# feiyuhuahuo/Yolact_minimal

Hardware: AMD Instinct MI355X
Metric: img/s res101_coco 544x544 inference (bs=1/GPU, 4 requests in flight) (higher is better)
Workload: dtype f32; 1 GPU; res101_coco 544x544 (the reference's "550-class" size) bs=1 inference: forward + nms + after_nms(480x640) per image, 4 independent bs=1 requests in flight on 4 HIP streams; global_batch=1, parallelism=replicas x1 (inference does not shard), weights=seeded random init, post_inputs=synthetic dense head outputs (17.8k candidates), requests_in_flight=4

## Files before the change

yolact_minimal_amd/csrc/conv_common.h:

```cpp
#pragma once
#include <cstdlib>
#include "ym_common.h"

namespace ymk {

constexpr int BK = 32;

struct FastDiv {
    unsigned mg, sh, d;
    __host__ static FastDiv make(unsigned d) {
        if (d == 0) d = 1;
        unsigned s = 0;
        while ((1ull << s) < d) ++s;
        return FastDiv{(unsigned)(((1ull << 32) * ((1ull << s) - d)) / d + 1), s, d};
    }
    __device__ __forceinline__ unsigned div(unsigned x) const { return (__umulhi(x, mg) + x) >> sh; }
    __device__ __forceinline__ void divmod(unsigned x, unsigned& q, unsigned& r) const { q = div(x); r = x - q * d; }
};

typedef int i32x4_t __attribute__((ext_vector_type(4)));
constexpr unsigned OOB = 0xFFFFFFF0u;
__device__ __forceinline__ f32x4 buf_ld16(__amdgpu_buffer_rsrc_t r, unsigned byte_off) {
    return __builtin_bit_cast(f32x4, __builtin_amdgcn_raw_buffer_load_b128(r, (int)byte_off, 0, 0));
}
__device__ __forceinline__ f32x4 buf_ld16_s(__amdgpu_buffer_rsrc_t r, unsigned byte_off, int soffset) {
    return __builtin_bit_cast(f32x4, __builtin_amdgcn_raw_buffer_load_b128(r, (int)byte_off, soffset, 0));
}
template <int I> struct IC { static constexpr int value = I; };
template <int I, int N, class F>
__device__ __forceinline__ void static_for(F&& f) {
    if constexpr (I < N) { f(IC<I>{}); static_for<I + 1, N>(f); }
}
constexpr int AUX_SC1 = 16;
__device__ __forceinline__ f32x4 buf_ld16_sc1(__amdgpu_buffer_rsrc_t r, unsigned byte_off) {
    return __builtin_bit_cast(f32x4, __builtin_amdgcn_raw_buffer_load_b128(r, (int)byte_off, 0, AUX_SC1));
}
__device__ __forceinline__ void buf_st16_sc1(__amdgpu_buffer_rsrc_t r, unsigned byte_off, f32x4 v) {
    __builtin_amdgcn_raw_buffer_store_b128(__builtin_bit_cast(i32x4_t, v), r, (int)byte_off, 0, AUX_SC1);
}

struct SegDev {
    float* out;
    long long bstride;
    int n0, n1, pitch, act;
};

struct ConvP {
    const float* in;
    const float* w;
    const float* scale;
    const float* shift;
    const float* residual;
    float* ws;
    double* bn_sum;
    double* bn_sumsq;
    const float* bnb_y;
    const float* bnb_out;
    const float* bnb_mean;
    const float* bnb_invstd;
    const float* bnb_gamma;
    const float* bnb_beta;
    int bnb_relu;
    int bn_ordered;
    int* counters;
    int B, H, W, Cin, Cout, KH, KW, stride, pad, Ho, Wo, Kpad;
    int M, HoWo, nkt, ksplit, kt_per_split, tiles_m, tiles_n;
    int main_blocks, main_tiles, tail_split, tail_ktps;
    FastDiv fd_ksplit, fd_tail, fd_tiles_n, fd_howo, fd_wo, fd_cin, fd_kw;
    int nlev;
    int lev_h[5], lev_w[5], lev_m[6], lev_pix[6];
    int cls;
    int M_pix;
    int cls_tile0[5];
    int cls_rows[4];
    int cls_w[4];
    FastDiv cls_fd_hw[4], cls_fd_w[4];
    int cls_kh0[4], cls_kw0[4], cls_nkw[4];
    int cls_nkt[4], cls_ktps[4], cls_tail_ktps[4];
    int n_groups;
    FastDiv fd_grp, fd_gn, fd_gn_last;
    long long* trace;
    const int* trace_epoch;
    int trace_ring;
    int trace_stride;
    int trace_rt;
    int* trace_hw;
    unsigned in_bytes, w_bytes, ws_bytes;
    int total_items;
    int nseg;
    int vec;
    SegDev seg[3];
};

__device__ __forceinline__ void ym_tile_decode(const ConvP& p, int id, int& tile_m, int& tile_n) {
    const unsigned g = p.fd_grp.div((unsigned)id);
    const unsigned r = (unsigned)id - g * p.fd_grp.d;
    const bool last = (int)g == p.n_groups - 1;
    const unsigned w = last ? p.fd_gn_last.d : p.fd_gn.d;
    const unsigned tm = last ? p.fd_gn_last.div(r) : p.fd_gn.div(r);
    tile_m = (int)tm;
    tile_n = (int)(g * p.fd_gn.d + (r - tm * w));
}

inline void ym_set_tile_order(ConvP& p, int groups, bool allow_model) {
    const int tn = p.tiles_n > 0 ? p.tiles_n : 1, tm = p.tiles_m > 0 ? p.tiles_m : 1;
    static const char* env = getenv("YM_TILE_GROUPS");
    if (groups <= 0) {
        const double a = (double)p.in_bytes, w = (double)p.w_bytes;
        if (env && env[0] == 'l') groups = (allow_model && w > a) ? tn : 1;
        else if (env && atoi(env) > 0) groups = allow_model ? atoi(env) : 1;
        else {
            groups = 1;
            double best = a + 8.0 * w;
            const bool small = a + w <= 8.0 * 1024 * 1024;
            if (allow_model && !small && w > a) groups = tn;
            for (int g = 2; g <= 8 && allow_model && small; g *= 2) {
                if (tn < g) break;
                const double t = g * a + (8.0 / g) * w;
                if (t < 0.95 * best) { best = t; groups = g; }
            }
        }
    }
    if (groups > tn) groups = tn;
    const int gw = (tn + groups - 1) / groups;
    p.n_groups = (tn + gw - 1) / gw;
    p.fd_gn = FastDiv::make((unsigned)gw);
    p.fd_gn_last = FastDiv::make((unsigned)(tn - (p.n_groups - 1) * gw));
    p.fd_grp = FastDiv::make((unsigned)(tm * gw));
}

#ifdef YM_TRACE
__device__ __forceinline__ size_t ym_trace_region(const ConvP& p) {
    if (!p.trace_epoch) return 0;
    const unsigned e = (unsigned)__hip_atomic_load(p.trace_epoch, __ATOMIC_RELAXED, __HIP_MEMORY_SCOPE_AGENT);
    return (size_t)(e % (unsigned)p.trace_ring) * (p.trace_stride ? (unsigned)p.trace_stride : gridDim.x);
}
#define YM_STAMP(i) do { if ((i) == 3) __builtin_amdgcn_s_waitcnt(0); if (p.trace && threadIdx.x == 0) { const size_t reg_ = ym_trace_region(p); p.trace[(reg_ + blockIdx.x) * 4 + (i)] = (long long)((p.trace_epoch || p.trace_rt) ? __builtin_amdgcn_s_memrealtime() : __builtin_amdgcn_s_memtime()) | ((i) == 0 ? (long long)(__builtin_amdgcn_s_getreg(0x1814) & 15) << 60 : 0ll); if ((i) == 0 && p.trace_hw) p.trace_hw[reg_ + blockIdx.x] = (int)__builtin_amdgcn_s_getreg(0xF804); } } while (0)
#else
#define YM_STAMP(i) do { } while (0)
#endif


__device__ __forceinline__ void row_to_image_pixel(const ConvP& p, int m, int& b, int& pix) {
    if (p.nlev > 0) {
        int base = 0, hw = p.lev_h[0] * p.lev_w[0], pix0 = 0;
#pragma unroll
        for (int q = 1; q < 5; ++q)
            if (q < p.nlev && m >= p.lev_m[q]) { base = p.lev_m[q]; hw = p.lev_h[q] * p.lev_w[q]; pix0 = p.lev_pix[q]; }
        const int local = m - base;
        b = local / hw;
        pix = pix0 + (local - b * hw);
    } else {
        b = (int)p.fd_howo.div((unsigned)m);
        pix = m - b * p.HoWo;
    }
}

__device__ __forceinline__ void epilogue_store(const ConvP& p, int m, int n, float acc) {
    float v = acc;
    v = __builtin_fmaf(v, p.scale ? p.scale[n] : 1.f, p.shift ? p.shift[n] : 0.f);
    if (p.residual) v += p.residual[(size_t)m * p.Cout + n];
    int b, pix;
    row_to_image_pixel(p, m, b, pix);
#pragma unroll
    for (int s = 0; s < 3; ++s) {
        if (s < p.nseg && n >= p.seg[s].n0 && n < p.seg[s].n1) {
            const SegDev& g = p.seg[s];
            g.out[(size_t)b * g.bstride + (size_t)pix * g.pitch + (n - g.n0)] = ym_apply_act(v, g.act);
        }
    }
}


enum ConvFamily { CONV_IGEMM, CONV_WAVE, CONV_WAVE_DMA, CONV_WS, CONV_PERS };
struct Plan {
    int bm, bn, ksplit, kt_per_split, tiles_m, tiles_n, nkt, M;
    int tail_tiles, tail_split, tail_ktps;
    int cls, M_pix, cls_tile0[5], cls_rows[4], cls_w[4], cls_hw[4], cls_kh0[4], cls_kw0[4], cls_nkw[4], cls_nkt[4];
    int kwaves;
    int family;
    int ring = 2;
    int mode = 0, spl = 0;
    bool dl = false, pf = false, pyramid = false;
    int grid_wgs;
    int pers_grid;
    bool pers_defer;
    bool vec, counters, fuses_bn;
    int bn_rows;
    int slots() const { return tail_tiles > 0 && tail_split > ksplit ? tail_split : ksplit; }
    size_t ws_bytes(int cout) const {
        const size_t u = ksplit > 1 ? (size_t)ksplit * M * cout * sizeof(float) : 0;
        const size_t t = tail_tiles > 0 ? (size_t)tail_tiles * tail_split * bm * bn * sizeof(float) : 0;
        return u > t ? u : t;
    }
    int grid() const { return (tiles_m * tiles_n - tail_tiles) * ksplit + tail_tiles * (tail_tiles > 0 ? tail_split : 0); }
    int stages() const {
        return ring + (family == CONV_PERS ? 40 : family == CONV_WS ? 50 : family == CONV_WAVE_DMA ? 20 : dl ? (pf ? 30 : 20) : 0);
    }
};

}

int ym_conv_plan(const ym_conv_desc* d, bool ws_aligned, ymk::Plan* pl);
int ym_cu_count();
int ym_launch_conv_wave(const ymk::ConvP& p, int tm, int tn, int kwaves, int ring, int waves_per_block, hipStream_t st);
int ym_launch_conv_pers(const ymk::ConvP& p, int bm, int bn, int mode, int ns, bool defer, int grid, hipStream_t st);
size_t ym_conv_pers_lds_bytes(int bm, int bn, int ns, bool defer);
int ym_launch_conv_ws(const ymk::ConvP& p, int bm, int bn, int nstg, int grid_wgs, hipStream_t st);
int ym_conv_ws_partial_rows(int M, int Cout, int bm, int bn, int nkt, int nstg, int grid_wgs);
size_t ym_conv_ws_lds_bytes(int bm, int bn, int nkt, int nstg);
```

yolact_minimal_amd/csrc/conv_mfma.hip:

```cpp
#include <stdlib.h>
#include <type_traits>
#include "conv_common.h"

using namespace ymk;

namespace {

constexpr int PITCH = 36;

template <int BM, int BN, int MODE, int NS, bool DL = false, bool PF = false, bool RG = false, int SPL = 0>
__global__ __launch_bounds__(256) void conv_igemm_f32(const ConvP p) {
    static_assert(SPL == 0 || (SPL <= 3 && !DL && !PF && (NS == 2 || NS == 3) && MODE != 1), "split-bf16: register staging, Cin % 32 == 0");
    constexpr int LB = SPL ? 2 : NS;
    constexpr int TM = BM / 64, TN = BN / 64;
    constexpr int AR = BM / 32, BR = BN / 32;
    constexpr int BP = 40;
    constexpr int RP = SPL ? (SPL * BP) / 2 : (DL ? 32 : PITCH);
    extern __shared__ __attribute__((aligned(16))) float smem[];
    float* As = smem;
    float* Bs = smem + LB * BM * RP;

    const int tid = threadIdx.x;
    const int lane = tid & 63, wave = __builtin_amdgcn_readfirstlane(tid >> 6);
    const int wm = wave >> 1, wn = wave & 1;
    YM_STAMP(0);
    const __amdgpu_buffer_rsrc_t rs_in = __builtin_amdgcn_make_buffer_rsrc((void*)p.in, 0, p.in_bytes, 0x00020000);
    const __amdgpu_buffer_rsrc_t rs_w = __builtin_amdgcn_make_buffer_rsrc((void*)p.w, 0, p.w_bytes, 0x00020000);
    const __amdgpu_buffer_rsrc_t rs_ws = __builtin_amdgcn_make_buffer_rsrc((void*)p.ws, 0, p.ws_bytes, 0x00020000);

    int id, ks, nks, ktps;
    {
        unsigned q, r;
        if ((int)blockIdx.x < p.main_blocks) {
            p.fd_ksplit.divmod((unsigned)ym_xcd_remap(blockIdx.x, p.main_blocks), q, r);
            id = (int)q; ks = (int)r;
            nks = p.ksplit; ktps = p.kt_per_split;
        } else {
            p.fd_tail.divmod(blockIdx.x - (unsigned)p.main_blocks, q, r);
            id = p.main_tiles + (int)q; ks = (int)r;
            nks = p.tail_split; ktps = p.tail_ktps;
        }
    }
    int tile_m, tile_n;
    ym_tile_decode(p, id, tile_m, tile_n);
    const int m0 = tile_m * BM, n0 = tile_n * BN;

    int cls = 0, cls_base = 0, c_kh0 = 0, c_kw0 = 0, c_step = 1, c_nkw = 1;
    bool cls_on = false;
    int kt_beg = ks * ktps, kt_end = min(p.nkt, kt_beg + ktps);
    if constexpr (MODE == 2) {
        if (p.cls) {
            cls_on = true;
            cls = tile_m & 3;
            cls_base = m0 - (tile_m >> 2) * BM;
            c_kh0 = p.cls_kh0[cls]; c_kw0 = p.cls_kw0[cls]; c_nkw = p.cls_nkw[cls]; c_step = 2;
            const int per = (int)blockIdx.x < p.main_blocks ? p.cls_ktps[cls] : p.cls_tail_ktps[cls];
            kt_beg = ks * per;
            kt_end = min(p.cls_nkt[cls], kt_beg + per);
        }
    }
    auto row_coords = [&](int m, int& b, int& oh, int& ow) __attribute__((always_inline)) -> bool {
        if (MODE == 2 && cls_on) {
            const int local = m - cls_base;
            if (local >= p.cls_rows[cls]) return false;
            unsigned ub, urem, ui, uj;
            p.cls_fd_hw[cls].divmod((unsigned)local, ub, urem);
            p.cls_fd_w[cls].divmod(urem, ui, uj);
            b = (int)ub; oh = 2 * (int)ui + (cls >> 1); ow = 2 * (int)uj + (cls & 1);
            return true;
        }
        if (m >= p.M) return false;
        unsigned ub, urem, uoh, uow;
        p.fd_howo.divmod((unsigned)m, ub, urem);
        p.fd_wo.divmod(urem, uoh, uow);
        b = (int)ub; oh = (int)uoh; ow = (int)uow;
        return true;
    };
    auto out_row = [&](int row) __attribute__((always_inline)) -> int {
        const int m = m0 + row;
        if (MODE == 2 && cls_on) {
            int b, oh, ow;
            return row_coords(m, b, oh, ow) ? (b * p.Ho + oh) * p.Wo + ow : -1;
        }
        return m < p.M ? m : -1;
    };

    const int c4 = DL ? ((tid & 7) ^ ((tid >> 4) & 7)) : (tid & 7);
    const int rbase = tid >> 3;
    int a_pix[AR];
    int a_ih0[AR], a_iw0[AR];
    int a_h[RG ? AR : 1], a_w[RG ? AR : 1];
#pragma unroll
    for (int i = 0; i < AR; ++i) {
        const int m = m0 + rbase + 32 * i;
        if constexpr (MODE == 2) {
            int b, oh, ow;
            if (row_coords(m, b, oh, ow)) {
                a_ih0[i] = oh + p.pad;
                a_iw0[i] = ow + p.pad;
                a_pix[i] = b * p.H;
            } else {
                a_ih0[i] = -(1 << 20);
                a_iw0[i] = -(1 << 20);
                a_pix[i] = 0;
            }
            continue;
        }
        if (m < p.M) {
            if constexpr (RG) {
                int base = 0, h = p.lev_h[0], w = p.lev_w[0];
#pragma unroll
                for (int q = 1; q < 5; ++q)
                    if (q < p.nlev && m >= p.lev_m[q]) { base = p.lev_m[q]; h = p.lev_h[q]; w = p.lev_w[q]; }
                const int local = m - base, hw = h * w;
                const int b = local / hw, rem = local - b * hw;
                const int oh = rem / w, ow = rem - oh * w;
                a_ih0[i] = oh - p.pad;
                a_iw0[i] = ow - p.pad;
                a_pix[i] = base + (b * h + a_ih0[i]) * w + a_iw0[i];
                a_h[i] = h; a_w[i] = w;
                continue;
            }
            unsigned ub, urem, uoh, uow;
            p.fd_howo.divmod((unsigned)m, ub, urem);
            p.fd_wo.divmod(urem, uoh, uow);
            const int b = (int)ub, oh = (int)uoh, ow = (int)uow;
            if (MODE == 2) {
                a_ih0[i] = oh + p.pad;
                a_iw0[i] = ow + p.pad;
                a_pix[i] = b * p.H;
            } else {
                a_ih0[i] = oh * p.stride - p.pad;
                a_iw0[i] = ow * p.stride - p.pad;
                a_pix[i] = (b * p.H + a_ih0[i]) * p.W + a_iw0[i];
            }
        } else {
            a_ih0[i] = -(1 << 20);
            a_iw0[i] = -(1 << 20);
            a_pix[i] = 0;
            if constexpr (RG) { a_h[i] = 1; a_w[i] = 1; }
        }
    }
    unsigned wrow[BR];
#pragma unroll
    for (int i = 0; i < BR; ++i) {
        const int n = n0 + rbase + 32 * i;
        wrow[i] = (n < p.Cout) ? (unsigned)((n * p.Kpad + c4 * 4) * 4) : p.w_bytes;
    }

    int kh = 0, kw = 0, c0 = 0;
    if (MODE == 0 || MODE == 2) {
        unsigned tap, uc0, ukh, ukw;
        p.fd_cin.divmod((unsigned)(kt_beg * BK), tap, uc0);
        c0 = (int)uc0;
        if (MODE == 2 && cls_on) {
            const int a = (int)tap / c_nkw;
            kh = c_kh0 + 2 * a; kw = c_kw0 + 2 * ((int)tap - a * c_nkw);
        } else {
            p.fd_kw.divmod(tap, ukh, ukw);
            kh = (int)ukh; kw = (int)ukw;
        }
    }

    unsigned a_off[AR];
    bool tap_dirty = true;
    int w_koff = 0;
    auto gather_tile = [&](int kt, auto&& sink_a, auto&& sink_b) __attribute__((always_inline)) {
        if (MODE == 0 || MODE == 2) {
            if (tap_dirty) {
                tap_dirty = false;
#pragma unroll
                for (int i = 0; i < AR; ++i) {
                    if (MODE == 0) {
                        const int ih = a_ih0[i] + kh, iw = a_iw0[i] + kw;
                        const int Hh = RG ? a_h[RG ? i : 0] : p.H, Ww = RG ? a_w[RG ? i : 0] : p.W;
                        const bool ok = (unsigned)ih < (unsigned)Hh && (unsigned)iw < (unsigned)Ww;
                        a_off[i] = (unsigned)(((a_pix[i] + kh * Ww + kw) * p.Cin + c4 * 4) * 4) | (ok ? 0u : OOB);
                    } else {
                        const int sh = p.stride >> 1, smask = p.stride - 1;
                        const int th = a_ih0[i] - kh, tw = a_iw0[i] - kw;
                        const int yh = th >> sh, yw = tw >> sh;
                        const bool ok = th >= 0 && tw >= 0 && ((th | tw) & smask) == 0 && yh < p.H && yw < p.W;
                        a_off[i] = (unsigned)((((a_pix[i] + yh) * p.W + yw) * p.Cin + c4 * 4) * 4) | (ok ? 0u : OOB);
                    }
                }
            }
#pragma unroll
            for (int i = 0; i < AR; ++i) sink_a(i, a_off[i], c0 * 4);
            if constexpr (MODE == 2) w_koff = ((kh * p.KW + kw) * p.Cin + c0) * 4;
            c0 += BK;
            if (c0 >= p.Cin) {
                c0 = 0;
                if constexpr (MODE == 2) { kw += c_step; if (kw >= p.KW) { kw = c_kw0; kh += c_step; } }
                else if (++kw == p.KW) { kw = 0; ++kh; }
                tap_dirty = true;
            }
        } else {
            const int tap = kt * 8 + c4;
            const int th = (int)p.fd_kw.div((unsigned)tap), tw = tap - th * p.KW;
            const bool tap_ok = tap < p.KH * p.KW;
#pragma unroll
            for (int i = 0; i < AR; ++i) {
                const int ih = a_ih0[i] + th, iw = a_iw0[i] + tw;
                const bool ok = tap_ok && (unsigned)ih < (unsigned)p.H && (unsigned)iw < (unsigned)p.W;
                const unsigned off = (unsigned)((a_pix[i] + th * p.W + tw) * 16);
                sink_a(i, ok ? off : OOB, 0);
            }
        }
#pragma unroll
        for (int i = 0; i < BR; ++i) sink_b(i, wrow[i], MODE == 2 ? w_koff : kt * BK * 4);
    };
    constexpr int NSET = (NS == 3 && !DL) ? 2 : 1;
    f32x4 rA[NSET][DL ? 1 : AR], rB[NSET][DL ? 1 : BR];
    auto load_tile = [&](int kt, auto set_c) __attribute__((always_inline)) {
        constexpr int SET = decltype(set_c)::value;
        gather_tile(kt, [&](int i, unsigned off, int soff) { rA[SET][DL ? 0 : i] = buf_ld16_s(rs_in, off, soff); },
                    [&](int i, unsigned off, int soff) { rB[SET][DL ? 0 : i] = buf_ld16_s(rs_w, off, soff); });
    };
    auto split_store = [&](unsigned short* row, const f32x4 v, int plane_stride) {
        typedef __bf16 bf16x2_t __attribute__((ext_vector_type(2)));
        typedef float f32x2_t __attribute__((ext_vector_type(2)));
        f32x4 r = v;
#pragma unroll
        for (int pl = 0; pl < (SPL ? SPL : 1); ++pl) {
            const unsigned p01 = __builtin_bit_cast(unsigned, __builtin_convertvector(f32x2_t{r[0], r[1]}, bf16x2_t));
            const unsigned p23 = __builtin_bit_cast(unsigned, __builtin_convertvector(f32x2_t{r[2], r[3]}, bf16x2_t));
            *reinterpret_cast<uint2*>(row + pl * plane_stride) = uint2{p01, p23};
            if (pl + 1 < SPL) {
                r[0] -= __uint_as_float(p01 << 16);
                r[1] -= __uint_as_float(p01 & 0xFFFF0000u);
                r[2] -= __uint_as_float(p23 << 16);
                r[3] -= __uint_as_float(p23 & 0xFFFF0000u);
            }
        }
    };
    auto store_tile = [&](int buf, auto set_c) __attribute__((always_inline)) {
        constexpr int SET = decltype(set_c)::value;
        float* a = As + buf * BM * RP;
        float* b = Bs + buf * BN * RP;
        if constexpr (SPL > 0) {
#pragma unroll
            for (int i = 0; i < AR; ++i)
                split_store(reinterpret_cast<unsigned short*>(a) + (rbase + 32 * i) * BP + c4 * 4, rA[SET][i], BM * BP);
#pragma unroll
            for (int i = 0; i < BR; ++i)
                split_store(reinterpret_cast<unsigned short*>(b) + (rbase + 32 * i) * BP + c4 * 4, rB[SET][i], BN * BP);
            return;
        }
#pragma unroll
        for (int i = 0; i < AR; ++i)
            *reinterpret_cast<f32x4*>(a + (rbase + 32 * i) * RP + c4 * 4) = rA[SET][DL ? 0 : i];
#pragma unroll
        for (int i = 0; i < BR; ++i)
            *reinterpret_cast<f32x4*>(b + (rbase + 32 * i) * RP + c4 * 4) = rB[SET][DL ? 0 : i];
    };
    auto dma_tile = [&](int kt, int buf) __attribute__((always_inline)) {
        typedef __attribute__((address_space(3))) void* lds_ptr;
        float* a = As + (buf * BM + 8 * wave) * RP;
        float* b = Bs + (buf * BN + 8 * wave) * RP;
        gather_tile(kt, [&](int i, unsigned off, int soff) { __builtin_amdgcn_raw_ptr_buffer_load_lds(rs_in, (lds_ptr)(a + 32 * i * RP), 16, (int)off, soff, 0, 0); },
                    [&](int i, unsigned off, int soff) { __builtin_amdgcn_raw_ptr_buffer_load_lds(rs_w, (lds_ptr)(b + 32 * i * RP), 16, (int)off, soff, 0, 0); });
    };

    f32x16 acc[TM][TN];
#pragma unroll
    for (int i = 0; i < TM; ++i)
#pragma unroll
        for (int j = 0; j < TN; ++j)
#pragma unroll
            for (int r = 0; r < 16; ++r) acc[i][j][r] = 0.f;

    constexpr bool DUAL = TM * TN == 1 && SPL == 0;
    f32x16 acc_odd;
#pragma unroll
    for (int r = 0; r < 16; ++r) acc_odd[r] = 0.f;

    const int frag_row = lane & 31, khalf = lane >> 5;
    const int a_frag_off = (wm * (BM / 2) + frag_row) * RP;
    const int b_frag_off = (wn * (BN / 2) + frag_row) * RP;
    int goff[4];
#pragma unroll
    for (int g = 0; g < 4; ++g) goff[g] = DL ? (((2 * g + khalf) ^ ((frag_row >> 1) & 7)) * 4) : (g * 8 + khalf * 4);

    auto compute = [&](int buf) __attribute__((always_inline)) {
        if constexpr (SPL > 0) {
            typedef __bf16 bf16x8_t __attribute__((ext_vector_type(8)));
            const unsigned short* a = reinterpret_cast<const unsigned short*>(As + buf * BM * RP) + (wm * (BM / 2) + frag_row) * BP + khalf * 8;
            const unsigned short* b = reinterpret_cast<const unsigned short*>(Bs + buf * BN * RP) + (wn * (BN / 2) + frag_row) * BP + khalf * 8;
#pragma unroll
            for (int kb = 0; kb < 2; ++kb) {
                bf16x8_t fa[TM][SPL], fb[TN][SPL];
#pragma unroll
                for (int i = 0; i < TM; ++i)
#pragma unroll
                    for (int pl = 0; pl < SPL; ++pl)
                        fa[i][pl] = *reinterpret_cast<const bf16x8_t*>(a + i * 32 * BP + pl * BM * BP + kb * 16);
#pragma unroll
                for (int j = 0; j < TN; ++j)
#pragma unroll
                    for (int pl = 0; pl < SPL; ++pl)
                        fb[j][pl] = *reinterpret_cast<const bf16x8_t*>(b + j * 32 * BP + pl * BN * BP + kb * 16);
#pragma unroll
                for (int sig = SPL - 1; sig >= 0; --sig)
#pragma unroll
                    for (int pa = 0; pa <= sig; ++pa)
#pragma unroll
                        for (int i = 0; i < TM; ++i)
#pragma unroll
                            for (int j = 0; j < TN; ++j)
                                acc[i][j] = __builtin_amdgcn_mfma_f32_32x32x16_bf16(fa[i][pa], fb[j][sig - pa], acc[i][j], 0, 0, 0);
            }
            return;
        }
        const float* a = As + buf * BM * RP + a_frag_off;
        const float* b = Bs + buf * BN * RP + b_frag_off;
#pragma unroll
        for (int g = 0; g < 4; ++g) {
            f32x4 fa[TM], fb[TN];
#pragma unroll
            for (int i = 0; i < TM; ++i) fa[i] = *reinterpret_cast<const f32x4*>(a + i * 32 * RP + goff[g]);
#pragma unroll
            for (int j = 0; j < TN; ++j) fb[j] = *reinterpret_cast<const f32x4*>(b + j * 32 * RP + goff[g]);
#pragma unroll
            for (int s = 0; s < 4; ++s) {
                if constexpr (DUAL) {
                    if (s & 1) acc_odd = __builtin_amdgcn_mfma_f32_32x32x2f32(fa[0][s], fb[0][s], acc_odd, 0, 0, 0);
                    else acc[0][0] = __builtin_amdgcn_mfma_f32_32x32x2f32(fa[0][s], fb[0][s], acc[0][0], 0, 0, 0);
                } else {
#pragma unroll
                    for (int i = 0; i < TM; ++i)
#pragma unroll
                        for (int j = 0; j < TN; ++j)
                            acc[i][j] = __builtin_amdgcn_mfma_f32_32x32x2f32(fa[i][s], fb[j][s], acc[i][j], 0, 0, 0);
                }
            }
        }
    };
    constexpr int EC4 = BN / 4, ERPP = 256 / EC4, ENR = BM / ERPP;
    constexpr bool PRE_RES = BM * BN <= 64 * 128;
    const bool direct = p.vec && nks == 1;
    f32x4 pre_sc = {1.f, 1.f, 1.f, 1.f}, pre_sh = {0.f, 0.f, 0.f, 0.f}, pre_res[PRE_RES ? ENR : 1];
    if (direct) {
        const int ecol4 = tid % EC4, erow0 = tid / EC4, en = n0 + ecol4 * 4;
        if (en < p.Cout) {
            if (p.scale) pre_sc = *reinterpret_cast<const f32x4*>(p.scale + en);
            if (p.shift) pre_sh = *reinterpret_cast<const f32x4*>(p.shift + en);
        }
        if (PRE_RES) {
            const __amdgpu_buffer_rsrc_t rs_res =
                __builtin_amdgcn_make_buffer_rsrc((void*)p.residual, 0, p.residual ? (unsigned)((size_t)p.M_pix * p.Cout * 4) : 0u, 0x00020000);
#pragma unroll
            for (int k = 0; k < ENR; ++k) {
                const int m = out_row(erow0 + k * ERPP);
                pre_res[k] = buf_ld16(rs_res, (m >= 0 && en < p.Cout) ? (unsigned)(((size_t)m * p.Cout + en) * 4) : OOB);
            }
        }
    }
    using I0 = std::integral_constant<int, 0>;
    using I1 = std::integral_constant<int, (NS == 3 && !DL) ? 1 : 0>;
    if constexpr (DL && PF) {
        static_assert(NS >= 3, "fragment prefetch needs a ring of 3+");
        constexpr int D = NS - 1;
        static_assert((AR + BR) * (D - 2) < 16, "vmcnt field");
        constexpr int WAIT = 0x070 | ((AR + BR) * (D - 2));
        const int nt = kt_end - kt_beg;
        auto read_frag = [&](int buf, int g, f32x4 (&fa)[TM], f32x4 (&fb)[TN]) __attribute__((always_inline)) {
            const float* a = As + buf * BM * RP + a_frag_off + goff[g];
            const float* b = Bs + buf * BN * RP + b_frag_off + goff[g];
#pragma unroll
            for (int i = 0; i < TM; ++i) fa[i] = *reinterpret_cast<const f32x4*>(a + i * 32 * RP);
#pragma unroll
            for (int j = 0; j < TN; ++j) fb[j] = *reinterpret_cast<const f32x4*>(b + j * 32 * RP);
        };
        auto mfma_group = [&](const f32x4 (&fa)[TM], const f32x4 (&fb)[TN]) __attribute__((always_inline)) {
#pragma unroll
            for (int s4 = 0; s4 < 4; ++s4) {
                if constexpr (DUAL) {
                    if (s4 & 1) acc_odd = __builtin_amdgcn_mfma_f32_32x32x2f32(fa[0][s4], fb[0][s4], acc_odd, 0, 0, 0);
                    else acc[0][0] = __builtin_amdgcn_mfma_f32_32x32x2f32(fa[0][s4], fb[0][s4], acc[0][0], 0, 0, 0);
                } else {
#pragma unroll
                    for (int i = 0; i < TM; ++i)
#pragma unroll
                        for (int j = 0; j < TN; ++j)
                            acc[i][j] = __builtin_amdgcn_mfma_f32_32x32x2f32(fa[i][s4], fb[j][s4], acc[i][j], 0, 0, 0);
                }
            }
        };
#pragma unroll
        for (int d = 0; d < D; ++d) dma_tile(kt_beg + d, d);
        __builtin_amdgcn_s_waitcnt(WAIT);
        __builtin_amdgcn_s_barrier();
        YM_STAMP(1);
        f32x4 fa0[TM], fb0[TN], fa1[TM], fb1[TN];
        read_frag(0, 0, fa0, fb0);
        auto tile = [&](auto S, int t) __attribute__((always_inline)) {
            constexpr int buf = decltype(S)::value, buf1 = (buf + 1) % NS, nb = (buf + D) % NS;
            dma_tile(kt_beg + t + D, nb);
            read_frag(buf, 1, fa1, fb1);
            __builtin_amdgcn_sched_barrier(0);
            mfma_group(fa0, fb0);
            __builtin_amdgcn_sched_barrier(0);
            read_frag(buf, 2, fa0, fb0);
            __builtin_amdgcn_sched_barrier(0);
            mfma_group(fa1, fb1);
            __builtin_amdgcn_sched_barrier(0);
            read_frag(buf, 3, fa1, fb1);
            __builtin_amdgcn_sched_barrier(0);
            mfma_group(fa0, fb0);
            __builtin_amdgcn_sched_barrier(0);
            read_frag(buf1, 0, fa0, fb0);
            __builtin_amdgcn_sched_barrier(0);
            mfma_group(fa1, fb1);
            __builtin_amdgcn_s_waitcnt(WAIT);
            __builtin_amdgcn_s_barrier();
        };
        int t = 0;
        for (; t + NS <= nt; t += NS) static_for<0, NS>([&](auto S) __attribute__((always_inline)) { tile(S, t + decltype(S)::value); });
        static_for<0, NS - 1>([&](auto S) __attribute__((always_inline)) { if (t + decltype(S)::value < nt) tile(S, t + decltype(S)::value); });
        __builtin_amdgcn_s_waitcnt(0xF70);
        __builtin_amdgcn_s_barrier();
    } else if constexpr (DL) {
        constexpr int D = NS - 1;
        static_assert((AR + BR) * (D - 1) < 16, "vmcnt field");
        constexpr int WAIT = 0x070 | ((AR + BR) * (D - 1));
        const int nt = kt_end - kt_beg;
#pragma unroll
        for (int d = 0; d < D; ++d) dma_tile(kt_beg + d, d);
        __builtin_amdgcn_s_waitcnt(WAIT);
        __builtin_amdgcn_s_barrier();
        YM_STAMP(1);
        auto tile = [&](auto S, int t) __attribute__((always_inline)) {
            constexpr int buf = decltype(S)::value, nb = (buf + D) % NS;
            dma_tile(kt_beg + t + D, nb);
            compute(buf);
            __builtin_amdgcn_s_waitcnt(WAIT);
            __builtin_amdgcn_s_barrier();
        };
        int t = 0;
        for (; t + NS <= nt; t += NS) static_for<0, NS>([&](auto S) __attribute__((always_inline)) { tile(S, t + decltype(S)::value); });
        static_for<0, NS - 1>([&](auto S) __attribute__((always_inline)) { if (t + decltype(S)::value < nt) tile(S, t + decltype(S)::value); });
        __builtin_amdgcn_s_waitcnt(0xF70);
        __builtin_amdgcn_s_barrier();
    } else if constexpr (NS == 3) {
        const int nt = kt_end - kt_beg;
        load_tile(kt_beg, I0{});
        store_tile(0, I0{});
        load_tile(kt_beg + 1, I1{});
        __syncthreads();
        YM_STAMP(1);
        int buf = 0;
        auto interleave = [&]() {
            if constexpr (SPL > 0) {
                constexpr int NMFMA = TM * TN * 2 * (SPL == 2 ? 3 : 6);
                constexpr int VPER = (SPL == 2 ? 12 : 24) * (AR + BR) / NMFMA + 1;
#pragma unroll
                for (int g = 0; g < NMFMA; ++g) {
                    __builtin_amdgcn_sched_group_barrier(0x008, 1, 0);
                    __builtin_amdgcn_sched_group_barrier(0x002, VPER, 0);
                }
            }
        };
        for (int t = 0; t < nt; t += 2) {
            load_tile(kt_beg + t + 2, I0{});
            compute(buf);
            int nb = buf == LB - 1 ? 0 : buf + 1;
            store_tile(nb, I1{});
            interleave();
            __syncthreads();
            buf = nb;
            if (t + 1 >= nt) break;
            load_tile(kt_beg + t + 3, I1{});
            compute(buf);
            nb = buf == LB - 1 ? 0 : buf + 1;
            store_tile(nb, I0{});
            interleave();
            __syncthreads();
            buf = nb;
        }
    } else {
        load_tile(kt_beg, I0{});
        store_tile(0, I0{});
        __syncthreads();
        YM_STAMP(1);
        auto tile = [&](auto S, int kt) __attribute__((always_inline)) {
            constexpr int cur = decltype(S)::value;
            load_tile(kt + 1, I0{});
            compute(cur);
            store_tile(cur ^ 1, I0{});
            __syncthreads();
        };
        int kt = kt_beg;
        for (; kt + 2 <= kt_end; kt += 2) { tile(IC<0>{}, kt); tile(IC<1>{}, kt + 1); }
        if (kt < kt_end) tile(IC<0>{}, kt);
    }

    if constexpr (DUAL) acc[0][0] += acc_odd;
    YM_STAMP(2);
    if (p.vec) {
        constexpr int CP = BN + 4;
        constexpr int C4 = BN / 4;
        constexpr int RPP = 256 / C4;
        float* C = smem;
#ifdef YM_TRACE
        const bool epi_abl = p.bnb_relu == 9 && p.bn_sum == nullptr;
        if (!epi_abl) {
#else
        constexpr bool epi_abl = false;
        {
#endif
#pragma unroll
            for (int j = 0; j < TN; ++j)
#pragma unroll
                for (int i = 0; i < TM; ++i)
#pragma unroll
                    for (int r = 0; r < 16; ++r)
                        C[(wm * (BM / 2) + i * 32 + 4 * khalf + (r & 3) + 8 * (r >> 2)) * CP + wn * (BN / 2) + j * 32 + frag_row] =
                            acc[i][j][r];
            __syncthreads();
        }
        const int col4 = tid % C4, row0 = tid / C4;
        const int n = n0 + col4 * 4;
        double bsum[4] = {0.0, 0.0, 0.0, 0.0}, bsq[4] = {0.0, 0.0, 0.0, 0.0};
        const size_t slice = (size_t)p.M * p.Cout;
        const bool in_tail = (int)blockIdx.x >= p.main_blocks;
        const unsigned sb = in_tail ? (unsigned)(BM * BN * 4) : (unsigned)(slice * 4);
        const unsigned rs = in_tail ? (unsigned)(BN * 4) : (unsigned)(p.Cout * 4);
        const unsigned ws0 = in_tail ? (unsigned)(id - p.main_tiles) * (unsigned)nks * sb + (unsigned)(col4 * 16)
                                     : (unsigned)m0 * rs + (unsigned)(n * 4);
        if (nks > 1) {
            const bool fused = p.counters != nullptr;
            if (n < p.Cout) {
                const unsigned base = ws0 + (unsigned)ks * sb;
#pragma unroll 4
                for (int row = row0; row < BM; row += RPP) {
                    const int m = m0 + row;
                    if (m < p.M) {
                        const f32x4 v = *reinterpret_cast<const f32x4*>(C + row * CP + col4 * 4);
                        if (fused) buf_st16_sc1(rs_ws, base + (unsigned)row * rs, v);
                        else *reinterpret_cast<f32x4*>(p.ws + (size_t)ks * slice + n + (size_t)m * p.Cout) = v;
                    }
                }
            }
            if (!fused) return;
            int& s_last = *reinterpret_cast<int*>(smem);
            asm volatile("s_waitcnt vmcnt(0)" ::: "memory");
            __syncthreads();
            if (tid == 0) {
                int* cnt = p.counters + tile_m * p.tiles_n + tile_n;
                const int old = __hip_atomic_fetch_add(cnt, 1, __ATOMIC_RELAXED, __HIP_MEMORY_SCOPE_AGENT);
                s_last = old == nks - 1;
                if (s_last) __hip_atomic_store(cnt, 0, __ATOMIC_RELAXED, __HIP_MEMORY_SCOPE_AGENT);
            }
            __syncthreads();
            if (!s_last) { YM_STAMP(3); return; }
        }
        if (n < p.Cout) {
            f32x4 sc = pre_sc, sh = pre_sh;
            if (!direct) {
                if (p.scale) sc = *reinterpret_cast<const f32x4*>(p.scale + n);
                if (p.shift) sh = *reinterpret_cast<const f32x4*>(p.shift + n);
            }
            const int act = p.seg[0].act;
            float* outb = p.seg[0].out + n;
            const bool fwd_stats = p.bn_sum != nullptr && p.bnb_y == nullptr;
            const float* resb = (p.residual && !(direct && PRE_RES)) ? p.residual + n : nullptr;
#pragma unroll
            for (int rk = 0; rk < BM / RPP; ++rk) {
                const int row = row0 + rk * RPP;
                const int m = out_row(row);
                if (m >= 0) {
                    f32x4 v;
                    if (nks > 1) {
                        const unsigned off = ws0 + (unsigned)row * rs;
                        v = buf_ld16_sc1(rs_ws, off);
                        int s2 = 1;
                        for (; s2 + 3 < nks; s2 += 4) {
                            const f32x4 a = buf_ld16_sc1(rs_ws, off + (unsigned)s2 * sb), b = buf_ld16_sc1(rs_ws, off + (unsigned)(s2 + 1) * sb);
                            const f32x4 c = buf_ld16_sc1(rs_ws, off + (unsigned)(s2 + 2) * sb), d = buf_ld16_sc1(rs_ws, off + (unsigned)(s2 + 3) * sb);
                            v += a; v += b; v += c; v += d;
                        }
                        for (; s2 < nks; ++s2) v += buf_ld16_sc1(rs_ws, off + (unsigned)s2 * sb);
                    } else if (epi_abl) {
                        v = f32x4{acc[0][0][(4 * rk) & 15], acc[0][0][(4 * rk + 1) & 15], acc[0][0][(4 * rk + 2) & 15], acc[0][0][(4 * rk + 3) & 15]};
                    } else {
                        v = *reinterpret_cast<const f32x4*>(C + row * CP + col4 * 4);
                    }
                    v = __builtin_elementwise_fma(v, sc, sh);
                    if (direct && PRE_RES) v += pre_res[PRE_RES ? rk : 0];
                    else if (resb) v += *reinterpret_cast<const f32x4*>(resb + (size_t)m * p.Cout);
#pragma unroll
                    for (int e = 0; e < 4; ++e) v[e] = ym_apply_act(v[e], act);
                    *reinterpret_cast<f32x4*>(outb + (size_t)m * p.Cout) = v;
                    if (fwd_stats) {
#pragma unroll
                        for (int e = 0; e < 4; ++e) { const double dv = v[e]; bsum[e] += dv; bsq[e] += dv * dv; }
                    }
                }
            }
            if (p.bnb_y) {
                const f32x4 b_mu = *reinterpret_cast<const f32x4*>(p.bnb_mean + n), b_is = *reinterpret_cast<const f32x4*>(p.bnb_invstd + n);
                f32x4 b_g = {1.f, 1.f, 1.f, 1.f}, b_bt = {0.f, 0.f, 0.f, 0.f};
                const bool remask = p.bnb_relu && !p.bnb_out;
                if (remask) { b_g = *reinterpret_cast<const f32x4*>(p.bnb_gamma + n); b_bt = *reinterpret_cast<const f32x4*>(p.bnb_beta + n); }
                constexpr int NR = BM / RPP, UR = 2;
#pragma unroll 1
                for (int rk0 = 0; rk0 < NR; rk0 += UR) {
                    f32x4 dv[UR], yy[UR], o[UR];
                    int mrow[UR];
#pragma unroll
                    for (int u = 0; u < UR; ++u) {
                        const int m = mrow[u] = out_row(row0 + (rk0 + u) * RPP);
                        const size_t off = (size_t)(m >= 0 ? m : 0) * p.Cout + n;
                        dv[u] = *reinterpret_cast<const f32x4*>(p.seg[0].out + off);
                        yy[u] = *reinterpret_cast<const f32x4*>(p.bnb_y + off);
                        if (p.bnb_out) o[u] = *reinterpret_cast<const f32x4*>(p.bnb_out + off);
                    }
#pragma unroll
                    for (int u = 0; u < UR; ++u) {
                        if (mrow[u] < 0) continue;
                        if (!p.bnb_out) {
#pragma unroll
                            for (int e = 0; e < 4; ++e) o[u][e] = remask ? bn_affine(yy[u][e], b_mu[e], b_is[e], b_g[e], b_bt[e]) : 1.f;
                        }
#pragma unroll
                        for (int e = 0; e < 4; ++e) {
                            const double dd = o[u][e] > 0.f ? dv[u][e] : 0.f;
                            bsum[e] += dd;
                            bsq[e] += dd * (double)((yy[u][e] - b_mu[e]) * b_is[e]);
                        }
                    }
                }
            }
        }
        if (p.bn_sum) {
            __syncthreads();
            double* R = reinterpret_cast<double*>(smem);
#pragma unroll
            for (int e = 0; e < 4; ++e) {
                R[((row0 * BN) + col4 * 4 + e) * 2 + 0] = bsum[e];
                R[((row0 * BN) + col4 * 4 + e) * 2 + 1] = bsq[e];
            }
            __syncthreads();
            if (tid < BN && n0 + tid < p.Cout) {
                double S = 0.0, Q = 0.0;
#pragma unroll
                for (int r = 0; r < RPP; ++r) { S += R[(r * BN + tid) * 2]; Q += R[(r * BN + tid) * 2 + 1]; }
                if (p.bn_ordered) {
                    double* row = p.bn_sum + (size_t)tile_m * 2 * p.Cout;
                    row[n0 + tid] = S;
                    row[p.Cout + n0 + tid] = Q;
                } else {
                    atomicAdd(p.bn_sum + n0 + tid, S);
                    atomicAdd(p.bn_sumsq + n0 + tid, Q);
                }
            }
        }
        YM_STAMP(3);
        return;
    }
    int* rowinfo = reinterpret_cast<int*>(smem);
    __syncthreads();
    if (tid < BM) {
        int b = 0, pix = 0;
        if (m0 + tid < p.M) row_to_image_pixel(p, m0 + tid, b, pix);
        rowinfo[2 * tid] = b;
        rowinfo[2 * tid + 1] = pix;
    }
    __syncthreads();
#pragma unroll
    for (int j = 0; j < TN; ++j) {
        const int n = n0 + wn * (BN / 2) + j * 32 + frag_row;
        const bool n_ok = n < p.Cout;
        float sc = 1.f, sh = 0.f;
        float* optr = nullptr;
        long long obs = 0;
        int opitch = 0, oact = 0;
        if (n_ok) {
            if (p.scale) sc = p.scale[n];
            if (p.shift) sh = p.shift[n];
#pragma unroll
            for (int s = 0; s < 3; ++s) {
                if (s < p.nseg && n >= p.seg[s].n0 && n < p.seg[s].n1) {
                    optr = p.seg[s].out + (n - p.seg[s].n0);
                    obs = p.seg[s].bstride; opitch = p.seg[s].pitch; oact = p.seg[s].act;
                }
            }
        }
#pragma unroll
        for (int i = 0; i < TM; ++i) {
            const int mb = m0 + wm * (BM / 2) + i * 32 + 4 * khalf;
            if (p.ksplit > 1) {
#pragma unroll
                for (int r = 0; r < 16; ++r) {
                    const int m = mb + (r & 3) + 8 * (r >> 2);
                    if (n_ok && m < p.M) p.ws[((size_t)ks * p.M + m) * p.Cout + n] = acc[i][j][r];
                }
            } else if (optr) {
#pragma unroll
                for (int r = 0; r < 16; ++r) {
                    const int m = mb + (r & 3) + 8 * (r >> 2);
                    if (m < p.M) {
                        float v = __builtin_fmaf(acc[i][j][r], sc, sh);
                        if (p.residual) v += p.residual[(size_t)m * p.Cout + n];
                        const int row = m - m0;
                        optr[(size_t)rowinfo[2 * row] * obs + (size_t)rowinfo[2 * row + 1] * opitch] = ym_apply_act(v, oact);
                    }
                }
            }
            __builtin_amdgcn_sched_barrier(0);
        }
    }
}

__global__ __launch_bounds__(256) void conv_splitk_reduce(const ConvP p) {
    const size_t total = (size_t)p.M * p.Cout;
    if (p.vec) {
        const size_t total4 = total / 4;
        const int act = p.seg[0].act;
        for (size_t q = (size_t)blockIdx.x * 256 + threadIdx.x; q < total4; q += (size_t)gridDim.x * 256) {
            const size_t e = q * 4;
            f32x4 v = *reinterpret_cast<const f32x4*>(p.ws + e);
            for (int s = 1; s < p.ksplit; ++s) v += *reinterpret_cast<const f32x4*>(p.ws + (size_t)s * total + e);
            const int n = (int)(e % p.Cout);
            f32x4 sc = {1.f, 1.f, 1.f, 1.f}, sh = {0.f, 0.f, 0.f, 0.f};
            if (p.scale) sc = *reinterpret_cast<const f32x4*>(p.scale + n);
            if (p.shift) sh = *reinterpret_cast<const f32x4*>(p.shift + n);
            v = __builtin_elementwise_fma(v, sc, sh);
            if (p.residual) v += *reinterpret_cast<const f32x4*>(p.residual + e);
#pragma unroll
            for (int k = 0; k < 4; ++k) v[k] = ym_apply_act(v[k], act);
            *reinterpret_cast<f32x4*>(p.seg[0].out + e) = v;
        }
        return;
    }
    for (size_t e = (size_t)blockIdx.x * 256 + threadIdx.x; e < total; e += (size_t)gridDim.x * 256) {
        float v = 0.f;
        for (int s = 0; s < p.ksplit; ++s) v += p.ws[(size_t)s * total + e];
        const int m = (int)(e / p.Cout), n = (int)(e - (size_t)m * p.Cout);
        epilogue_store(p, m, n, v);
    }
}

template <int BM, int BN, int MODE, int NS = 2, bool DL = false, bool PF = false, bool RG = false, int SPL = 0>
void launch(const ConvP& p, int grid, hipStream_t st) {
    size_t lds = SPL ? (size_t)2 * (BM + BN) * SPL * 80 : (size_t)NS * (BM + BN) * (DL ? 32 : PITCH) * sizeof(float);
    const size_t epi = (size_t)BM * (BN + 4) * sizeof(float);
    if (lds < epi) lds = epi;
    static YmLdsAttr attr = {};
    (void)ym_ensure_dyn_lds(attr, reinterpret_cast<const void*>(conv_igemm_f32<BM, BN, MODE, NS, DL, PF, RG, SPL>), lds, "conv_igemm_f32");
    hipLaunchKernelGGL((conv_igemm_f32<BM, BN, MODE, NS, DL, PF, RG, SPL>), dim3(grid), dim3(256), lds, st, p);
}

bool launch_igemm(const ConvP& p, const Plan& pl, int grid, hipStream_t st) {
#define YM_V(BM_, BN_, MODE_, NS_, DL_, PF_, RG_, SPL_)                                                                               \
    if (pl.bm == BM_ && pl.bn == BN_ && pl.mode == MODE_ && pl.ring == NS_ && pl.dl == DL_ && pl.pf == PF_ && pl.pyramid == RG_ && \
        pl.spl == SPL_) { launch<BM_, BN_, MODE_, NS_, DL_, PF_, RG_, SPL_>(p, grid, st); return true; }
    YM_V(128, 128, 0, 2, 0, 0, 0, 0)
    YM_V(128, 128, 0, 2, 1, 0, 0, 0)
    YM_V(128, 128, 0, 3, 1, 0, 0, 0)
    YM_V(128,  64, 0, 2, 0, 0, 0, 0)
    YM_V(128,  64, 0, 3, 0, 0, 0, 0)
    YM_V(128,  64, 0, 2, 1, 0, 0, 0)
    YM_V(128,  64, 0, 3, 1, 0, 0, 0)
    YM_V( 64, 128, 0, 2, 0, 0, 0, 0)
    YM_V( 64, 128, 0, 3, 0, 0, 0, 0)
    YM_V( 64, 128, 0, 2, 1, 0, 0, 0)
    YM_V( 64, 128, 0, 3, 1, 0, 0, 0)
    YM_V( 64,  64, 0, 2, 0, 0, 0, 0)
    YM_V( 64,  64, 0, 3, 0, 0, 0, 0)
    YM_V( 64,  64, 0, 2, 1, 0, 0, 0)
    YM_V( 64,  64, 0, 3, 1, 0, 0, 0)
    YM_V( 64,  64, 0, 4, 1, 0, 0, 0)
    YM_V( 64,  64, 0, 3, 1, 1, 0, 0)
    YM_V( 64,  64, 0, 4, 1, 1, 0, 0)
    YM_V(128, 128, 2, 2, 0, 0, 0, 0)
    YM_V(128, 128, 2, 2, 1, 0, 0, 0)
    YM_V(128, 128, 2, 3, 1, 0, 0, 0)
    YM_V(128,  64, 2, 2, 0, 0, 0, 0)
    YM_V(128,  64, 2, 2, 1, 0, 0, 0)
    YM_V(128,  64, 2, 3, 1, 0, 0, 0)
    YM_V( 64, 128, 2, 2, 0, 0, 0, 0)
    YM_V( 64, 128, 2, 2, 1, 0, 0, 0)
    YM_V( 64, 128, 2, 3, 1, 0, 0, 0)
    YM_V( 64,  64, 2, 2, 0, 0, 0, 0)
    YM_V( 64,  64, 2, 3, 0, 0, 0, 0)
    YM_V( 64,  64, 2, 2, 1, 0, 0, 0)
    YM_V( 64,  64, 2, 3, 1, 0, 0, 0)
    YM_V(128,  64, 1, 2, 0, 0, 0, 0)
    YM_V(128, 128, 0, 2, 0, 0, 1, 0)
    YM_V(128,  64, 0, 2, 0, 0, 1, 0)
    YM_V( 64, 128, 0, 2, 0, 0, 1, 0)
    YM_V( 64,  64, 0, 2, 0, 0, 1, 0)
    YM_V(128, 128, 0, 2, 0, 0, 0, 2)
    YM_V(128, 128, 0, 3, 0, 0, 0, 2)
    YM_V(128,  64, 0, 2, 0, 0, 0, 2)
    YM_V(128,  64, 0, 3, 0, 0, 0, 2)
    YM_V( 64, 128, 0, 2, 0, 0, 0, 2)
    YM_V( 64, 128, 0, 3, 0, 0, 0, 2)
    YM_V( 64,  64, 0, 2, 0, 0, 0, 2)
    YM_V( 64,  64, 0, 3, 0, 0, 0, 2)
    YM_V(128, 128, 0, 2, 0, 0, 0, 3)
    YM_V(128, 128, 0, 3, 0, 0, 0, 3)
    YM_V(128,  64, 0, 2, 0, 0, 0, 3)
    YM_V(128,  64, 0, 3, 0, 0, 0, 3)
    YM_V( 64, 128, 0, 2, 0, 0, 0, 3)
    YM_V( 64, 128, 0, 3, 0, 0, 0, 3)
    YM_V( 64,  64, 0, 2, 0, 0, 0, 3)
    YM_V( 64,  64, 0, 3, 0, 0, 0, 3)
    YM_V(128, 128, 2, 2, 0, 0, 0, 2)
    YM_V(128, 128, 2, 3, 0, 0, 0, 2)
    YM_V(128,  64, 2, 2, 0, 0, 0, 2)
    YM_V(128,  64, 2, 3, 0, 0, 0, 2)
    YM_V( 64, 128, 2, 2, 0, 0, 0, 2)
    YM_V( 64, 128, 2, 3, 0, 0, 0, 2)
    YM_V( 64,  64, 2, 2, 0, 0, 0, 2)
    YM_V( 64,  64, 2, 3, 0, 0, 0, 2)
    YM_V(128, 128, 2, 2, 0, 0, 0, 3)
    YM_V(128, 128, 2, 3, 0, 0, 0, 3)
    YM_V(128,  64, 2, 2, 0, 0, 0, 3)
    YM_V(128,  64, 2, 3, 0, 0, 0, 3)
    YM_V( 64, 128, 2, 2, 0, 0, 0, 3)
    YM_V( 64, 128, 2, 3, 0, 0, 0, 3)
    YM_V( 64,  64, 2, 2, 0, 0, 0, 3)
    YM_V( 64,  64, 2, 3, 0, 0, 0, 3)
#undef YM_V
    return false;
}

int fill_params(const ym_conv_desc* d, const Plan& pl, void* workspace, ConvP& p) {
    const size_t need = pl.ws_bytes(d->Cout);
    p.in = d->in; p.w = d->weight; p.scale = d->scale; p.shift = d->shift; p.residual = d->residual;
    p.ws = (float*)workspace;
    p.B = d->B; p.H = d->H; p.W = d->W; p.Cin = d->Cin; p.Cout = d->Cout; p.KH = d->KH; p.KW = d->KW;
    p.stride = d->stride; p.pad = d->pad; p.Ho = d->Ho; p.Wo = d->Wo; p.Kpad = d->k_pad;
    {
        const unsigned long long ib = (d->nlevels ? (unsigned long long)pl.M : (unsigned long long)d->B * d->H * d->W) * d->Cin * 4ull, wb = (unsigned long long)d->Cout * d->k_pad * 4ull;
        YM_REQUIRE(ib < 0xFFFFFFF0ull && wb < 0x7FFFFFF0ull, "conv: input must be < 4 GiB and the packed weight < 2 GiB (32-bit buffer offsets)");
        p.in_bytes = (unsigned)ib; p.w_bytes = (unsigned)wb;
    }
    p.nlev = d->nlevels;
    {
        int m_acc = 0, pix_acc = 0;
        for (int l = 0; l < 5; ++l) {
            const bool on = l < d->nlevels;
            p.lev_h[l] = on ? d->level_h[l] : 1; p.lev_w[l] = on ? d->level_w[l] : 1;
            p.lev_m[l] = m_acc; p.lev_pix[l] = pix_acc;
            if (on) { m_acc += d->B * d->level_h[l] * d->level_w[l]; pix_acc += d->level_h[l] * d->level_w[l]; }
        }
        p.lev_m[5] = m_acc; p.lev_pix[5] = pix_acc;
    }
    p.M = pl.M; p.HoWo = d->Ho * d->Wo; p.nkt = pl.nkt; p.ksplit = pl.ksplit; p.kt_per_split = pl.kt_per_split;
    p.M_pix = pl.M_pix; p.cls = pl.cls;
    for (int c = 0; c < 4; ++c) {
        const bool on = pl.cls != 0;
        p.cls_tile0[c] = on ? pl.cls_tile0[c] : 0; p.cls_rows[c] = on ? pl.cls_rows[c] : 0; p.cls_w[c] = on ? pl.cls_w[c] : 1;
        p.cls_fd_hw[c] = FastDiv::make((unsigned)(on ? pl.cls_hw[c] : 1)); p.cls_fd_w[c] = FastDiv::make((unsigned)(on ? pl.cls_w[c] : 1));
        p.cls_kh0[c] = on ? pl.cls_kh0[c] : 0; p.cls_kw0[c] = on ? pl.cls_kw0[c] : 0; p.cls_nkw[c] = on ? pl.cls_nkw[c] : 1;
        p.cls_nkt[c] = on ? pl.cls_nkt[c] : 0;
        p.cls_ktps[c] = on ? ym_cdiv(pl.cls_nkt[c], pl.ksplit) : 0;
        p.cls_tail_ktps[c] = on && pl.tail_tiles > 0 ? ym_cdiv(pl.cls_nkt[c], pl.tail_split) : 0;
    }
    p.cls_tile0[4] = pl.cls ? pl.cls_tile0[4] : 0;
    p.tiles_m = pl.tiles_m; p.tiles_n = pl.tiles_n; p.nseg = d->nseg;
    for (int i = 0; i < 3; ++i) {
        if (i < d->nseg) {
            p.seg[i].out = d->seg[i].out; p.seg[i].bstride = d->seg[i].batch_stride; p.seg[i].n0 = d->seg[i].n_begin;
            p.seg[i].n1 = d->seg[i].n_end; p.seg[i].pitch = d->seg[i].pitch; p.seg[i].act = d->seg[i].act;
        } else {
            p.seg[i] = SegDev{nullptr, 0, 0, 0, 0, 0};
        }
    }
    YM_REQUIRE(pl.tail_tiles == 0 || ((uintptr_t)workspace & 15) == 0, "conv: tail split needs a 16-byte aligned workspace");
    p.vec = pl.vec;
    p.bn_sum = d->bn_sum; p.bn_sumsq = d->bn_sumsq; p.bn_ordered = (d->bn_sum && d->bn_ordered) ? 1 : 0;
    p.bnb_y = d->bnb_y; p.bnb_out = d->bnb_out; p.bnb_mean = d->bnb_mean; p.bnb_invstd = d->bnb_invstd;
    p.bnb_gamma = d->bnb_gamma; p.bnb_beta = d->bnb_beta; p.bnb_relu = d->bnb_relu;
    p.trace = nullptr; p.trace_epoch = nullptr; p.trace_ring = 0; p.trace_stride = 0; p.trace_rt = 0; p.trace_hw = nullptr;
#ifdef YM_TRACE
    if (const char* e = getenv("YM_TRACE_PTR")) p.trace = (long long*)strtoull(e, nullptr, 10);
    if (const char* e = getenv("YM_TRACE_EPOCH_PTR")) p.trace_epoch = (const int*)strtoull(e, nullptr, 10);
    if (const char* e = getenv("YM_TRACE_RING")) p.trace_ring = atoi(e);
    if (const char* e = getenv("YM_TRACE_GRID")) p.trace_stride = atoi(e);
    if (const char* e = getenv("YM_TRACE_REALTIME")) p.trace_rt = atoi(e);
    if (const char* e = getenv("YM_TRACE_HW_PTR")) p.trace_hw = (int*)strtoull(e, nullptr, 10);
    if (p.trace_ring <= 0) p.trace_epoch = nullptr;
    if (const char* e = getenv("YM_PERS_ABL")) { if (!d->bn_sum) p.bnb_relu = atoi(e); }
#endif
    p.counters = pl.counters ? d->tile_counters : nullptr;
    YM_REQUIRE(!pl.cls || (p.vec && (pl.slots() == 1 || p.counters)), "conv(dgrad, stride 2): the class-ordered plan needs a 16-byte aligned workspace");
    YM_REQUIRE(pl.tail_tiles == 0 || p.counters, "conv: tail_tiles needs a plain NHWC output (vector epilogue) and a workspace < 4 GiB");
    p.main_tiles = pl.tiles_m * pl.tiles_n - pl.tail_tiles;
    p.main_blocks = p.main_tiles * pl.ksplit;
    p.tail_split = pl.tail_tiles > 0 ? pl.tail_split : 1;
    p.tail_ktps = pl.tail_tiles > 0 ? pl.tail_ktps : pl.nkt;
    p.fd_ksplit = FastDiv::make((unsigned)pl.ksplit); p.fd_tail = FastDiv::make((unsigned)p.tail_split);
    p.fd_tiles_n = FastDiv::make((unsigned)pl.tiles_n);
    ym_set_tile_order(p, 0, pl.tail_tiles == 0);
    p.fd_howo = FastDiv::make((unsigned)(d->Ho * d->Wo));
    p.fd_wo = FastDiv::make((unsigned)d->Wo); p.fd_cin = FastDiv::make((unsigned)d->Cin); p.fd_kw = FastDiv::make((unsigned)d->KW);
    p.ws_bytes = (unsigned)(need < 0xFFFFFFF0ull ? need : 0);
    p.total_items = pl.grid();
    if (d->bn_sum) {
        YM_REQUIRE((d->bn_sumsq || d->bn_ordered) && ((uintptr_t)d->bn_sum & 7) == 0 && pl.fuses_bn,
                   "conv: bn_sum given but this configuration cannot fuse the statistics (ask ym_conv2d_fuses_bn_stats)");
    }
    if (d->bnb_y) {
        YM_REQUIRE(d->bn_sum && d->bnb_mean && d->bnb_invstd && (!d->bnb_relu || d->bnb_out || (d->bnb_gamma && d->bnb_beta)),
                   "conv: bnb_y needs bn_sum / bn_sumsq, bnb_mean, bnb_invstd and (with bnb_relu) bnb_out or bnb_gamma + bnb_beta");
        YM_REQUIRE(d->Cout % 4 == 0 && ((uintptr_t)d->bnb_y & 15) == 0 && ((uintptr_t)d->bnb_out & 15) == 0,
                   "conv: bnb_y / bnb_out must be 16-byte aligned [M][Cout] tensors");
    }
    YM_REQUIRE(pl.family != CONV_WAVE_DMA || (size_t)pl.M * d->Cout * 4 < 0xFFFFFFF0ull, "conv(wave, DMA ring): the output must be < 4 GiB");
    if (pl.family == CONV_IGEMM && d->mma != 0) {
        YM_REQUIRE(d->mma == 3 || d->mma == 6, "conv: mma must be 0 (f32 MFMA), 3 (bf16x3) or 6 (bf16x6), got %d", d->mma);
        YM_REQUIRE(d->nlevels == 0 && d->Cin % 32 == 0, "conv: split-bf16 mode needs Cin %% 32 == 0 and a single-size input");
    }
    return YM_OK;
}

int launch_plan(const ConvP& p, const Plan& pl, hipStream_t st) {
    switch (pl.family) {
        case CONV_WAVE: case CONV_WAVE_DMA: return ym_launch_conv_wave(p, pl.bm, pl.bn, pl.kwaves, pl.ring, pl.grid_wgs, st);
        case CONV_WS: return ym_launch_conv_ws(p, pl.bm, pl.bn, pl.ring, pl.grid_wgs, st);
        case CONV_PERS: return ym_launch_conv_pers(p, pl.bm, pl.bn, pl.mode, pl.ring, pl.pers_defer, pl.pers_grid, st);
    }
    if (!launch_igemm(p, pl, pl.grid(), st)) {
        ym_set_error("conv: no conv_igemm_f32<%d, %d, %d, %d, %d, %d, %d, %d> is built (planner bug)", pl.bm, pl.bn, pl.mode, pl.ring, pl.dl, pl.pf, pl.pyramid, pl.spl);
        return YM_EINVAL;
    }
    int rc = ym_check_launch("conv_igemm_f32");
    if (rc == YM_OK && pl.ksplit > 1 && !p.counters) {
        const size_t total = (size_t)p.M * p.Cout;
        int rgrid = (int)((total / (p.vec ? 4 : 1) + 255) / 256);
        if (rgrid > 2048) rgrid = 2048;
        hipLaunchKernelGGL(conv_splitk_reduce, dim3(rgrid), dim3(256), 0, st, p);
        rc = ym_check_launch("conv_splitk_reduce");
    }
    return rc;
}

}

extern "C" size_t ym_sizeof_conv_desc(void) { return sizeof(ym_conv_desc); }

extern "C" size_t ym_conv2d_workspace_bytes(const ym_conv_desc* d) {
    Plan pl;
    return ym_conv_plan(d, true, &pl) == YM_OK ? pl.ws_bytes(d->Cout) : 0;
}

extern "C" int ym_conv2d_tile_counters(const ym_conv_desc* d) {
    Plan pl;
    return ym_conv_plan(d, true, &pl) == YM_OK && pl.slots() > 1 ? pl.tiles_m * pl.tiles_n : 0;
}

extern "C" int ym_conv2d_fuses_bn_stats(const ym_conv_desc* d) {
    Plan pl;
    return ym_conv_plan(d, true, &pl) == YM_OK && pl.fuses_bn ? 1 : 0;
}

extern "C" int ym_conv2d_bn_partial_rows(const ym_conv_desc* d) {
    Plan pl;
    return ym_conv_plan(d, true, &pl) == YM_OK ? pl.bn_rows : 0;
}

extern "C" int ym_conv2d_effective_plan(const ym_conv_desc* d, int32_t out[8]) {
    Plan pl;
    YM_REQUIRE(out, "conv: effective_plan needs an output row");
    if (int rc = ym_conv_plan(d, true, &pl)) return rc;
    const bool tail = pl.tail_tiles > 0;
    const int32_t row[8] = {pl.bm, pl.bn, pl.ksplit, d->kwaves, pl.stages(), tail ? pl.tail_tiles : 0, tail ? pl.tail_split : 0, pl.grid_wgs};
    for (int i = 0; i < 8; ++i) out[i] = row[i];
    return YM_OK;
}

extern "C" int ym_conv2d_fwd(const ym_conv_desc* d, void* workspace, size_t workspace_bytes, ym_stream_t s) {
    Plan pl;
    if (int rc = ym_conv_plan(d, ((uintptr_t)workspace & 15) == 0, &pl)) return rc;
    const size_t need = pl.ws_bytes(d->Cout);
    if (need > workspace_bytes || (need && !workspace)) {
        ym_set_error("conv: workspace %zu B < %zu B needed (ksplit %d)", workspace_bytes, need, pl.ksplit);
        return YM_ENOSPC;
    }
    ConvP p;
    if (int rc = fill_params(d, pl, workspace, p)) return rc;
    if (d->bn_sum && !d->bn_ordered) ym_note_unordered_sum();
    return launch_plan(p, pl, (hipStream_t)s);
}
```

yolact_minimal_amd/csrc/conv_persist.hip:

```cpp
#include "conv_common.h"

using namespace ymk;

namespace {

constexpr int waitcnt_imm(int vm, int lgkm) { return (vm & 15) | ((vm >> 4) << 14) | (7 << 4) | ((lgkm & 15) << 8); }

__device__ __forceinline__ void wg_sync_lds() {
    asm volatile("s_waitcnt lgkmcnt(0)\n\ts_barrier" ::: "memory");
}

template <int BM, int BN, int MODE, int NS, bool DEFER, bool ALIGNED>
__global__ __launch_bounds__(256) void conv_igemm_pers(const ConvP p) {
    static_assert(BM == 64 && BN == 64, "the accumulator staging aliases one ring stage: (BM + BN) * 128 B == BM * BN * 4 B");
    static_assert(MODE == 0 || MODE == 2, "Cin % 32 == 0 convolution / data gradient");
    static_assert(NS >= 2 && NS <= 12, "ring depth");
    constexpr int AR = BM / 32, BR = BN / 32;
    constexpr int RP = 32;
    constexpr int D = NS - 1;
    constexpr int STAGE = (BM + BN) * RP;
    constexpr bool PF = NS >= 3;
    static_assert((AR + BR) * (D - 1) < 64, "vmcnt field");
    constexpr int WAIT = waitcnt_imm((AR + BR) * (PF ? D - 2 : D - 1), 0);
    extern __shared__ __attribute__((aligned(16))) float smem[];
    float* C2 = smem + NS * STAGE;
    int* s_flag = reinterpret_cast<int*>(smem + NS * STAGE + (DEFER ? BM * BN : 0));

    const int tid = threadIdx.x;
    const int lane = tid & 63, wave = __builtin_amdgcn_readfirstlane(tid >> 6);
    const int wm = wave >> 1, wn = wave & 1;
    const __amdgpu_buffer_rsrc_t rs_in = __builtin_amdgcn_make_buffer_rsrc((void*)p.in, 0, p.in_bytes, 0x00020000);
    const __amdgpu_buffer_rsrc_t rs_w = __builtin_amdgcn_make_buffer_rsrc((void*)p.w, 0, p.w_bytes, 0x00020000);
    const __amdgpu_buffer_rsrc_t rs_ws = __builtin_amdgcn_make_buffer_rsrc((void*)p.ws, 0, p.ws_bytes, 0x00020000);
    const __amdgpu_buffer_rsrc_t rs_res =
        __builtin_amdgcn_make_buffer_rsrc((void*)p.residual, 0, p.residual ? (unsigned)((size_t)p.M * p.Cout * 4) : 0u, 0x00020000);

    struct Item { int id, ks, nks, kt_beg, kt_end, tile_m, tile_n; };
    auto decode = [&](int b) __attribute__((always_inline)) {
        Item it;
        unsigned q, r;
        int ktps;
        if (b < p.main_blocks) {
            p.fd_ksplit.divmod((unsigned)ym_xcd_remap(b, p.main_blocks), q, r);
            it.id = (int)q; it.ks = (int)r; it.nks = p.ksplit; ktps = p.kt_per_split;
        } else {
            p.fd_tail.divmod((unsigned)(b - p.main_blocks), q, r);
            it.id = p.main_tiles + (int)q; it.ks = (int)r; it.nks = p.tail_split; ktps = p.tail_ktps;
        }
        ym_tile_decode(p, it.id, it.tile_m, it.tile_n);
        it.kt_beg = it.ks * ktps;
        it.kt_end = min(p.nkt, it.kt_beg + ktps);
        return it;
    };

    const int c4 = (tid & 7) ^ ((tid >> 4) & 7);
    const int rbase = tid >> 3;
    int a_pix[AR], a_ih0[AR], a_iw0[AR];
    unsigned wrow[BR], a_off[AR];
    int kh = 0, kw = 0, c0 = 0;
    bool tap_dirty = true;
    int ld_item = (int)blockIdx.x, ld_kt = 0, ld_end = 0;

    auto setup_loader = [&](int b) __attribute__((always_inline)) {
        tap_dirty = true;
        const bool live = b < p.total_items;
        const Item it = decode(live ? b : 0);
        const int m0 = it.tile_m * BM, n0 = it.tile_n * BN;
#pragma unroll
        for (int i = 0; i < AR; ++i) {
            const int m = m0 + rbase + 32 * i;
            if (live && m < p.M) {
                unsigned ub, urem, uoh, uow;
                p.fd_howo.divmod((unsigned)m, ub, urem);
                p.fd_wo.divmod(urem, uoh, uow);
                const int b_ = (int)ub, oh = (int)uoh, ow = (int)uow;
                if (MODE == 2) {
                    a_ih0[i] = oh + p.pad;
                    a_iw0[i] = ow + p.pad;
                    a_pix[i] = b_ * p.H;
                } else {
                    a_ih0[i] = oh * p.stride - p.pad;
                    a_iw0[i] = ow * p.stride - p.pad;
                    a_pix[i] = (b_ * p.H + a_ih0[i]) * p.W + a_iw0[i];
                }
            } else {
                a_ih0[i] = -(1 << 20);
                a_iw0[i] = -(1 << 20);
                a_pix[i] = 0;
            }
        }
#pragma unroll
        for (int i = 0; i < BR; ++i) {
            const int n = n0 + rbase + 32 * i;
            wrow[i] = (live && n < p.Cout) ? (unsigned)((n * p.Kpad + c4 * 4) * 4) : p.w_bytes;
        }
        unsigned tap, uc0, ukh, ukw;
        p.fd_cin.divmod((unsigned)(it.kt_beg * BK), tap, uc0);
        p.fd_kw.divmod(tap, ukh, ukw);
        c0 = (int)uc0; kh = (int)ukh; kw = (int)ukw;
        ld_kt = it.kt_beg; ld_end = live ? it.kt_end : 0x7FFFFFFF;
    };

    auto dma_next = [&](int stage) __attribute__((always_inline)) {
        typedef __attribute__((address_space(3))) void* lds_ptr;
        if (ld_kt == ld_end) {
            ld_item += (int)gridDim.x;
            setup_loader(ld_item);
        }
        if (tap_dirty) {
            tap_dirty = false;
#pragma unroll
            for (int i = 0; i < AR; ++i) {
                if (MODE == 0) {
                    const int ih = a_ih0[i] + kh, iw = a_iw0[i] + kw;
                    const bool ok = (unsigned)ih < (unsigned)p.H && (unsigned)iw < (unsigned)p.W;
                    a_off[i] = (unsigned)(((a_pix[i] + kh * p.W + kw) * p.Cin + c4 * 4) * 4) | (ok ? 0u : OOB);
                } else {
                    const int sh = p.stride >> 1, smask = p.stride - 1;
                    const int th = a_ih0[i] - kh, tw = a_iw0[i] - kw;
                    const int yh = th >> sh, yw = tw >> sh;
                    const bool ok = th >= 0 && tw >= 0 && ((th | tw) & smask) == 0 && yh < p.H && yw < p.W;
                    a_off[i] = (unsigned)((((a_pix[i] + yh) * p.W + yw) * p.Cin + c4 * 4) * 4) | (ok ? 0u : OOB);
                }
            }
        }
        float* a = smem + stage * STAGE + 8 * wave * RP;
        float* b = a + BM * RP;
#pragma unroll
        for (int i = 0; i < AR; ++i)
            __builtin_amdgcn_raw_ptr_buffer_load_lds(rs_in, (lds_ptr)(a + 32 * i * RP), 16, (int)a_off[i], c0 * 4, 0, 0);
#pragma unroll
        for (int i = 0; i < BR; ++i)
            __builtin_amdgcn_raw_ptr_buffer_load_lds(rs_w, (lds_ptr)(b + 32 * i * RP), 16, (int)wrow[i], ld_kt * BK * 4, 0, 0);
        ++ld_kt;
        c0 += BK;
        if (c0 >= p.Cin) {
            c0 = 0;
            if (++kw == p.KW) { kw = 0; ++kh; }
            tap_dirty = true;
        }
    };

    const int frag_row = lane & 31, khalf = lane >> 5;
    const int a_frag_off = (wm * 32 + frag_row) * RP;
    const int b_frag_off = BM * RP + (wn * 32 + frag_row) * RP;
    typedef const __attribute__((address_space(3))) f32x4* lds_frag_ptr;
    lds_frag_ptr pa[4], pb[4];
#pragma unroll
    for (int g = 0; g < 4; ++g) {
        const int goff = ((2 * g + khalf) ^ ((frag_row >> 1) & 7)) * 4;
        pa[g] = (lds_frag_ptr)(smem + a_frag_off + goff);
        pb[g] = (lds_frag_ptr)(smem + b_frag_off + goff);
    }
    f32x16 acc, acc_odd;

    auto compute = [&](int stage) __attribute__((always_inline)) {
#pragma unroll
        for (int g = 0; g < 4; ++g) {
            const f32x4 fa = pa[g][stage * (STAGE / 4)];
            const f32x4 fb = pb[g][stage * (STAGE / 4)];
            acc = __builtin_amdgcn_mfma_f32_32x32x2f32(fa[0], fb[0], acc, 0, 0, 0);
            acc_odd = __builtin_amdgcn_mfma_f32_32x32x2f32(fa[1], fb[1], acc_odd, 0, 0, 0);
            acc = __builtin_amdgcn_mfma_f32_32x32x2f32(fa[2], fb[2], acc, 0, 0, 0);
            acc_odd = __builtin_amdgcn_mfma_f32_32x32x2f32(fa[3], fb[3], acc_odd, 0, 0, 0);
        }
    };

    auto read_frag = [&](int stage, int g, f32x4& fa, f32x4& fb) __attribute__((always_inline)) {
        fa = pa[g][stage * (STAGE / 4)];
        fb = pb[g][stage * (STAGE / 4)];
    };
    auto mfma_group = [&](const f32x4& fa, const f32x4& fb) __attribute__((always_inline)) {
        acc = __builtin_amdgcn_mfma_f32_32x32x2f32(fa[0], fb[0], acc, 0, 0, 0);
        acc_odd = __builtin_amdgcn_mfma_f32_32x32x2f32(fa[1], fb[1], acc_odd, 0, 0, 0);
        acc = __builtin_amdgcn_mfma_f32_32x32x2f32(fa[2], fb[2], acc, 0, 0, 0);
        acc_odd = __builtin_amdgcn_mfma_f32_32x32x2f32(fa[3], fb[3], acc_odd, 0, 0, 0);
    };

    constexpr int C4 = BN / 4;
    constexpr int RPP = 256 / C4;
    constexpr int ENR = BM / RPP;
    const int col4 = tid % C4, row0 = tid / C4;
    const size_t slice = (size_t)p.M * p.Cout;
    const int act_relu = p.seg[0].act == YM_ACT_RELU;

    bool pend = false, c_dirty = false;
    int pend_m0 = 0, pend_n0 = 0;
    f32x4 pend_sc = {1.f, 1.f, 1.f, 1.f}, pend_sh = {0.f, 0.f, 0.f, 0.f}, pend_res[ENR];
    auto flush_pending = [&]() __attribute__((always_inline)) {
        const int pn = pend_n0 + col4 * 4;
        if (pn < p.Cout) {
            float* outb = p.seg[0].out + pn;
#pragma unroll
            for (int rk = 0; rk < ENR; ++rk) {
                const int row = row0 + rk * RPP;
                const int m = pend_m0 + row;
                if (m < p.M) {
                    f32x4 v = *reinterpret_cast<const f32x4*>(C2 + row * BN + col4 * 4);
                    v = __builtin_elementwise_fma(v, pend_sc, pend_sh);
                    v += pend_res[rk];
                    if (act_relu) {
#pragma unroll
                        for (int e = 0; e < 4; ++e) v[e] = v[e] < 0.f ? 0.f : v[e];
                    }
                    *reinterpret_cast<f32x4*>(outb + (size_t)m * p.Cout) = v;
                }
            }
        }
        pend = false;
        c_dirty = true;
    };

    setup_loader(ld_item);
#pragma unroll
    for (int d = 0; d < D; ++d) dma_next(d);
    __builtin_amdgcn_s_waitcnt(WAIT);
    __builtin_amdgcn_s_barrier();
    int buf = 0, nb = D;

    for (int bid = (int)blockIdx.x; bid < p.total_items; bid += (int)gridDim.x) {
        const Item it = decode(bid);
        const int m0 = it.tile_m * BM, n0 = it.tile_n * BN, nks = it.nks, ks = it.ks;
        const int n = n0 + col4 * 4;
        const bool direct = nks == 1;
        f32x4 pre_sc = {1.f, 1.f, 1.f, 1.f}, pre_sh = {0.f, 0.f, 0.f, 0.f}, pre_res[ENR];
        if (direct && !DEFER) {
            if (n < p.Cout) {
                if (p.scale) pre_sc = *reinterpret_cast<const f32x4*>(p.scale + n);
                if (p.shift) pre_sh = *reinterpret_cast<const f32x4*>(p.shift + n);
            }
#pragma unroll
            for (int k = 0; k < ENR; ++k) {
                const int m = m0 + row0 + k * RPP;
                pre_res[k] = buf_ld16(rs_res, (m < p.M && n < p.Cout) ? (unsigned)(((size_t)m * p.Cout + n) * 4) : OOB);
            }
        }
#pragma unroll
        for (int r = 0; r < 16; ++r) { acc[r] = 0.f; acc_odd[r] = 0.f; }
        const int nt = it.kt_end - it.kt_beg;
#ifdef YM_TRACE
        if (p.bnb_relu >= 1 && p.bnb_relu <= 5) {
            const f32x4 ra = {1.f, 2.f, 3.f, 4.f}, rb = {.5f, .25f, .125f, 1.f};
            for (int t = 0; t < nt; ++t) {
                if (p.bnb_relu == 1) dma_next(nb);
                else if (p.bnb_relu == 2) compute(buf);
                else {
#pragma unroll
                    for (int g = 0; g < 4; ++g) mfma_group(ra, rb);
                }
                if (p.bnb_relu != 5) {
                    __builtin_amdgcn_s_waitcnt(WAIT);
                    __builtin_amdgcn_s_barrier();
                }
                nb = buf;
                buf = buf == NS - 1 ? 0 : buf + 1;
                if constexpr (DEFER) {
                    if (t == 0) { if (pend) flush_pending(); } else c_dirty = false;
                }
            }
        } else
#endif
        if constexpr (ALIGNED && PF) {
            f32x4 fa0, fb0, fa1, fb1;
            read_frag(0, 0, fa0, fb0);
            auto tile = [&](auto SC, int t) __attribute__((always_inline)) {
                    constexpr int B0 = decltype(SC)::value, B1 = (B0 + 1) % NS, BP = (B0 + NS - 1) % NS;
                    dma_next(BP);
                    read_frag(B0, 1, fa1, fb1);
                    __builtin_amdgcn_sched_barrier(0);
                    mfma_group(fa0, fb0);
                    __builtin_amdgcn_sched_barrier(0);
                    read_frag(B0, 2, fa0, fb0);
                    __builtin_amdgcn_sched_barrier(0);
                    mfma_group(fa1, fb1);
                    __builtin_amdgcn_sched_barrier(0);
                    read_frag(B0, 3, fa1, fb1);
                    __builtin_amdgcn_sched_barrier(0);
                    mfma_group(fa0, fb0);
                    __builtin_amdgcn_sched_barrier(0);
                    if (B0 + 1 < NS || t + NS < nt) read_frag(B1, 0, fa0, fb0);
                    __builtin_amdgcn_sched_barrier(0);
                    mfma_group(fa1, fb1);
                    __builtin_amdgcn_s_waitcnt(WAIT);
                    __builtin_amdgcn_s_barrier();
            };
            for (int t = 0; t < nt; t += NS) {
                tile(IC<0>{}, t);
                if constexpr (DEFER) {
                    if (t == 0) { if (pend) flush_pending(); } else c_dirty = false;
                }
                static_for<1, NS>([&](auto SC) __attribute__((always_inline)) { tile(SC, t); });
                if constexpr (DEFER) c_dirty = false;
            }
        } else if constexpr (ALIGNED) {
            auto tile = [&](auto SC) __attribute__((always_inline)) {
                constexpr int B0 = decltype(SC)::value;
                dma_next((B0 + NS - 1) % NS);
                compute(B0);
                __builtin_amdgcn_s_waitcnt(WAIT);
                __builtin_amdgcn_s_barrier();
            };
            for (int t = 0; t < nt; t += NS) {
                tile(IC<0>{});
                if constexpr (DEFER) {
                    if (t == 0) { if (pend) flush_pending(); } else c_dirty = false;
                }
                static_for<1, NS>([&](auto SC) __attribute__((always_inline)) { tile(SC); });
                if constexpr (DEFER) c_dirty = false;
            }
        } else if constexpr (PF) {
            f32x4 fa0, fb0, fa1, fb1;
            read_frag(buf, 0, fa0, fb0);
            for (int t = 0; t < nt; ++t) {
                const int buf1 = buf == NS - 1 ? 0 : buf + 1;
                dma_next(nb);
                read_frag(buf, 1, fa1, fb1);
                __builtin_amdgcn_sched_barrier(0);
                mfma_group(fa0, fb0);
                __builtin_amdgcn_sched_barrier(0);
                read_frag(buf, 2, fa0, fb0);
                __builtin_amdgcn_sched_barrier(0);
                mfma_group(fa1, fb1);
                __builtin_amdgcn_sched_barrier(0);
                read_frag(buf, 3, fa1, fb1);
                __builtin_amdgcn_sched_barrier(0);
                mfma_group(fa0, fb0);
                __builtin_amdgcn_sched_barrier(0);
                if (t + 1 < nt) read_frag(buf1, 0, fa0, fb0);
                __builtin_amdgcn_sched_barrier(0);
                mfma_group(fa1, fb1);
                __builtin_amdgcn_s_waitcnt(WAIT);
                __builtin_amdgcn_s_barrier();
                nb = buf;
                buf = buf1;
                if constexpr (DEFER) {
                    if (t == 0) { if (pend) flush_pending(); } else c_dirty = false;
                }
            }
        } else {
            for (int t = 0; t < nt; ++t) {
                dma_next(nb);
                compute(buf);
                __builtin_amdgcn_s_waitcnt(WAIT);
                __builtin_amdgcn_s_barrier();
                nb = buf;
                buf = buf == NS - 1 ? 0 : buf + 1;
                if constexpr (DEFER) {
                    if (t == 0) { if (pend) flush_pending(); } else c_dirty = false;
                }
            }
        }
        acc += acc_odd;
        if (DEFER && direct) {
            if (c_dirty) wg_sync_lds();
#pragma unroll
            for (int r = 0; r < 16; ++r)
                C2[(wm * 32 + 4 * khalf + (r & 3) + 8 * (r >> 2)) * BN + wn * 32 + frag_row] = acc[r];
            pend_sc = f32x4{1.f, 1.f, 1.f, 1.f};
            pend_sh = f32x4{0.f, 0.f, 0.f, 0.f};
            if (n < p.Cout) {
                if (p.scale) pend_sc = *reinterpret_cast<const f32x4*>(p.scale + n);
                if (p.shift) pend_sh = *reinterpret_cast<const f32x4*>(p.shift + n);
            }
#pragma unroll
            for (int k = 0; k < ENR; ++k) {
                const int m = m0 + row0 + k * RPP;
                pend_res[k] = buf_ld16(rs_res, (m < p.M && n < p.Cout) ? (unsigned)(((size_t)m * p.Cout + n) * 4) : OOB);
            }
            pend_m0 = m0; pend_n0 = n0;
            pend = true;
            c_dirty = false;
            continue;
        }

        float* C = smem + nb * STAGE;
#pragma unroll
        for (int r = 0; r < 16; ++r)
            C[(wm * 32 + 4 * khalf + (r & 3) + 8 * (r >> 2)) * BN + wn * 32 + frag_row] = acc[r];
        wg_sync_lds();
        const bool in_tail = bid >= p.main_blocks;
        const unsigned sb = in_tail ? (unsigned)(BM * BN * 4) : (unsigned)(slice * 4);
        const unsigned rs = in_tail ? (unsigned)(BN * 4) : (unsigned)(p.Cout * 4);
        const unsigned ws0 = in_tail ? (unsigned)(it.id - p.main_tiles) * (unsigned)nks * sb + (unsigned)(col4 * 16)
                                     : (unsigned)m0 * rs + (unsigned)(n * 4);
        bool finish = true;
        if (nks > 1) {
            if (n < p.Cout) {
                const unsigned base = ws0 + (unsigned)ks * sb;
#pragma unroll
                for (int k = 0; k < ENR; ++k) {
                    const int row = row0 + k * RPP;
                    if (m0 + row < p.M) buf_st16_sc1(rs_ws, base + (unsigned)row * rs, *reinterpret_cast<const f32x4*>(C + row * BN + col4 * 4));
                }
            }
            asm volatile("s_waitcnt vmcnt(0)" ::: "memory");
            wg_sync_lds();
            if (tid == 0) {
                int* cnt = p.counters + it.tile_m * p.tiles_n + it.tile_n;
                const int old = __hip_atomic_fetch_add(cnt, 1, __ATOMIC_RELAXED, __HIP_MEMORY_SCOPE_AGENT);
                const int last = old == nks - 1;
                *s_flag = last;
                if (last) __hip_atomic_store(cnt, 0, __ATOMIC_RELAXED, __HIP_MEMORY_SCOPE_AGENT);
            }
            wg_sync_lds();
            finish = *s_flag != 0;
        }
        if (finish && n < p.Cout) {
            f32x4 sc = pre_sc, sh = pre_sh;
            if (!direct) {
                if (p.scale) sc = *reinterpret_cast<const f32x4*>(p.scale + n);
                if (p.shift) sh = *reinterpret_cast<const f32x4*>(p.shift + n);
            }
            float* outb = p.seg[0].out + n;
#pragma unroll
            for (int rk = 0; rk < ENR; ++rk) {
                const int row = row0 + rk * RPP;
                const int m = m0 + row;
                if (m < p.M) {
                    f32x4 v;
                    if (nks > 1) {
                        const unsigned off = ws0 + (unsigned)row * rs;
                        v = buf_ld16_sc1(rs_ws, off);
                        int s2 = 1;
                        for (; s2 + 3 < nks; s2 += 4) {
                            const f32x4 a = buf_ld16_sc1(rs_ws, off + (unsigned)s2 * sb), b = buf_ld16_sc1(rs_ws, off + (unsigned)(s2 + 1) * sb);
                            const f32x4 c = buf_ld16_sc1(rs_ws, off + (unsigned)(s2 + 2) * sb), d = buf_ld16_sc1(rs_ws, off + (unsigned)(s2 + 3) * sb);
                            v += a; v += b; v += c; v += d;
                        }
                        for (; s2 < nks; ++s2) v += buf_ld16_sc1(rs_ws, off + (unsigned)s2 * sb);
                    } else {
                        v = *reinterpret_cast<const f32x4*>(C + row * BN + col4 * 4);
                    }
                    v = __builtin_elementwise_fma(v, sc, sh);
                    if (direct) v += pre_res[rk];
                    else if (p.residual) v += *reinterpret_cast<const f32x4*>(p.residual + (size_t)m * p.Cout + n);
                    if (act_relu) {
#pragma unroll
                        for (int e = 0; e < 4; ++e) v[e] = v[e] < 0.f ? 0.f : v[e];
                    }
                    *reinterpret_cast<f32x4*>(outb + (size_t)m * p.Cout) = v;
                }
            }
        }
        wg_sync_lds();
    }
    if constexpr (DEFER) {
        if (pend) {
            wg_sync_lds();
            flush_pending();
        }
    }
    asm volatile("s_waitcnt vmcnt(0)" ::: "memory");
}

template <int BM, int BN, int MODE, int NS, bool DEFER, bool ALIGNED>
int launch_pers(const ConvP& p, int grid, hipStream_t st) {
    const size_t lds = ym_conv_pers_lds_bytes(BM, BN, NS, DEFER);
    static YmLdsAttr attr = {};
    if (int rc = ym_ensure_dyn_lds(attr, reinterpret_cast<const void*>(conv_igemm_pers<BM, BN, MODE, NS, DEFER, ALIGNED>), lds, "conv_igemm_pers")) return rc;
    hipLaunchKernelGGL((conv_igemm_pers<BM, BN, MODE, NS, DEFER, ALIGNED>), dim3(grid), dim3(256), lds, st, p);
    return ym_check_launch("conv_igemm_pers");
}

template <int MODE, bool DEFER>
int launch_pers_ns(const ConvP& p, int ns, int grid, hipStream_t st) {
    const bool main_ok = p.main_blocks == 0 || (p.nkt % ns == 0 && (p.ksplit == 1 || p.kt_per_split % ns == 0));
    const bool tail_ok = p.total_items == p.main_blocks || (p.nkt % ns == 0 && p.tail_ktps % ns == 0);
    const bool al = main_ok && tail_ok && ns <= 4;
    switch (ns) {
        case 2: return al ? launch_pers<64, 64, MODE, 2, DEFER, true>(p, grid, st) : launch_pers<64, 64, MODE, 2, DEFER, false>(p, grid, st);
        case 3: return al ? launch_pers<64, 64, MODE, 3, DEFER, true>(p, grid, st) : launch_pers<64, 64, MODE, 3, DEFER, false>(p, grid, st);
        case 4: return al ? launch_pers<64, 64, MODE, 4, DEFER, true>(p, grid, st) : launch_pers<64, 64, MODE, 4, DEFER, false>(p, grid, st);
        case 6: return launch_pers<64, 64, MODE, 6, DEFER, false>(p, grid, st);
        case 8: return launch_pers<64, 64, MODE, 8, DEFER, false>(p, grid, st);
        default: ym_set_error("conv(persistent): ring depth %d not built (2, 3, 4, 6, 8)", ns); return YM_EINVAL;
    }
}

}

size_t ym_conv_pers_lds_bytes(int bm, int bn, int ns, bool defer) {
    return (size_t)ns * (bm + bn) * 32 * sizeof(float) + (defer ? (size_t)bm * bn * sizeof(float) : 0) + 16;
}

int ym_launch_conv_pers(const ConvP& p, int bm, int bn, int mode, int ns, bool defer, int grid, hipStream_t st) {
    if (bm != 64 || bn != 64 || (mode != 0 && mode != 2)) {
        ym_set_error("conv(persistent): 64x64 tile, convolution or data gradient only (got %dx%d mode %d)", bm, bn, mode);
        return YM_EINVAL;
    }
    if (defer) return mode == 0 ? launch_pers_ns<0, true>(p, ns, grid, st) : launch_pers_ns<2, true>(p, ns, grid, st);
    return mode == 0 ? launch_pers_ns<0, false>(p, ns, grid, st) : launch_pers_ns<2, false>(p, ns, grid, st);
}
```

yolact_minimal_amd/csrc/conv_wave.hip:

```cpp
#include "conv_common.h"

using namespace ymk;

namespace {

constexpr int waitcnt_vm(int vm) { return (vm & 15) | ((vm >> 4) << 14) | (7 << 4) | (15 << 8); }

template <int N>
struct Frag {
    f32x4 v[N][4];
};

template <int TM, int TN, int KW, int WPB>
__device__ __forceinline__ void wave_tile_finish(const ConvP& p, float* slabs, f32x16 (&acc)[TM][TN], int wave, int lane, bool tile_ok,
                                                 int tile_local, int kslice, int m0, int n0) {
    constexpr int WM = 32 * TM, WN = 32 * TN;
    constexpr int CP = WN + 4;
    const int frag_row = lane & 31, khalf = lane >> 5;
    constexpr int C4_ = WN / 4, LANES_ = KW * 64, NPASS = (WM * C4_ + LANES_ - 1) / LANES_;
    f32x4 pre_res[NPASS];
    const bool pre = p.vec && p.residual != nullptr && tile_ok;
    if (pre) {
        const int lt_ = kslice * 64 + lane, col4_ = lt_ % C4_, row0_ = lt_ / C4_;
        const __amdgpu_buffer_rsrc_t rs_res = __builtin_amdgcn_make_buffer_rsrc((void*)p.residual, 0, (unsigned)((size_t)p.M * p.Cout * 4), 0x00020000);
#pragma unroll
        for (int k = 0; k < NPASS; ++k) {
            const int m = m0 + row0_ + k * (LANES_ / C4_), n = n0 + col4_ * 4;
            pre_res[k] = buf_ld16(rs_res, (row0_ + k * (LANES_ / C4_) < WM && m < p.M && n < p.Cout) ? (unsigned)(((size_t)m * p.Cout + n) * 4) : OOB);
        }
    }
    float* mine = slabs + (size_t)wave * WM * CP;
#pragma unroll
    for (int j = 0; j < TN; ++j)
#pragma unroll
        for (int i = 0; i < TM; ++i)
#pragma unroll
            for (int r = 0; r < 16; ++r)
                mine[(i * 32 + 4 * khalf + (r & 3) + 8 * (r >> 2)) * CP + j * 32 + frag_row] = acc[i][j][r];
    __syncthreads();
    if (!tile_ok) return;
    const float* slab0 = slabs + (size_t)(tile_local * KW) * WM * CP;
    constexpr int C4 = WN / 4;
    constexpr int LANES = KW * 64;
    const int lt = kslice * 64 + lane;
    if (p.vec) {
        const int col4 = lt % C4, row0 = lt / C4;
        const int n = n0 + col4 * 4;
        if (n < p.Cout) {
            f32x4 sc = {1.f, 1.f, 1.f, 1.f}, sh = {0.f, 0.f, 0.f, 0.f};
            if (p.scale) sc = *reinterpret_cast<const f32x4*>(p.scale + n);
            if (p.shift) sh = *reinterpret_cast<const f32x4*>(p.shift + n);
            const int act = p.seg[0].act;
#pragma unroll
            for (int k = 0; k < NPASS; ++k) {
                const int row = row0 + k * (LANES / C4);
                const int m = m0 + row;
                if (row >= WM || m >= p.M) break;
                f32x4 v = *reinterpret_cast<const f32x4*>(slab0 + row * CP + col4 * 4);
#pragma unroll
                for (int s = 1; s < KW; ++s) v += *reinterpret_cast<const f32x4*>(slab0 + (size_t)s * WM * CP + row * CP + col4 * 4);
                v = __builtin_elementwise_fma(v, sc, sh);
                if (p.residual) v += pre_res[k];
#pragma unroll
                for (int e = 0; e < 4; ++e) v[e] = ym_apply_act(v[e], act);
                *reinterpret_cast<f32x4*>(p.seg[0].out + (size_t)m * p.Cout + n) = v;
            }
        }
    } else {
        for (int e = lt; e < WM * WN; e += LANES) {
            const int row = e / WN, col = e - row * WN;
            const int m = m0 + row, n = n0 + col;
            if (m < p.M && n < p.Cout) {
                float v = slab0[row * CP + col];
#pragma unroll
                for (int s = 1; s < KW; ++s) v += slab0[(size_t)s * WM * CP + row * CP + col];
                epilogue_store(p, m, n, v);
            }
        }
    }
}

template <int TM, int TN, int KW, int WPB>
__global__ __launch_bounds__(WPB * 64) void conv_wave_f32(const ConvP p) {
    constexpr int TPB = WPB / KW;
    constexpr int WM = 32 * TM, WN = 32 * TN;
    constexpr int D = 3;
    extern __shared__ __attribute__((aligned(16))) float smem[];

    const int lane = threadIdx.x & 63;
    const int wave = __builtin_amdgcn_readfirstlane(threadIdx.x >> 6);
    const int tile_local = wave / KW, kslice = wave - tile_local * KW;
    const int frag_row = lane & 31, khalf = lane >> 5;

    const int bid = ym_xcd_remap(blockIdx.x, gridDim.x);
    const int tile = bid * TPB + tile_local;
    const int ntiles = p.tiles_m * p.tiles_n;
    const bool tile_ok = tile < ntiles;
    const int tile_m = tile_ok ? tile / p.tiles_n : 0, tile_n = tile_ok ? tile - tile_m * p.tiles_n : 0;
    const int m0 = tile_m * WM, n0 = tile_n * WN;

    int a_pix[TM], a_ih0[TM], a_iw0[TM];
#pragma unroll
    for (int i = 0; i < TM; ++i) {
        const int m = m0 + i * 32 + frag_row;
        if (tile_ok && m < p.M) {
            const int b = m / p.HoWo, rem = m - b * p.HoWo;
            const int oh = rem / p.Wo, ow = rem - oh * p.Wo;
            a_ih0[i] = oh * p.stride - p.pad;
            a_iw0[i] = ow * p.stride - p.pad;
            a_pix[i] = (b * p.H + a_ih0[i]) * p.W + a_iw0[i];
        } else {
            a_ih0[i] = -(1 << 20); a_iw0[i] = -(1 << 20); a_pix[i] = 0;
        }
    }
    const float* wrow[TN];
#pragma unroll
    for (int j = 0; j < TN; ++j) {
        const int n = n0 + j * 32 + frag_row;
        wrow[j] = (tile_ok && n < p.Cout) ? p.w + (size_t)n * p.Kpad + khalf * 4 : nullptr;
    }

    const int nt = tile_ok ? (p.nkt - kslice + KW - 1) / KW : 0;
    int kh, kw, c0;
    {
        const int k0 = kslice * BK;
        const int tap = k0 / p.Cin;
        c0 = k0 - tap * p.Cin;
        kh = tap / p.KW;
        kw = tap - kh * p.KW;
    }
    int kt_next = kslice;

    Frag<TM> fa[D];
    Frag<TN> fb[D];
    auto load_tile = [&](Frag<TM>& A, Frag<TN>& Bf) {
        const int tap_off = kh * p.W + kw;
#pragma unroll
        for (int i = 0; i < TM; ++i) {
            const int ih = a_ih0[i] + kh, iw = a_iw0[i] + kw;
            const bool ok = (unsigned)ih < (unsigned)p.H && (unsigned)iw < (unsigned)p.W;
            if (ok) {
                const float* src = p.in + (size_t)(a_pix[i] + tap_off) * p.Cin + c0 + khalf * 4;
#pragma unroll
                for (int g = 0; g < 4; ++g) A.v[i][g] = *reinterpret_cast<const f32x4*>(src + g * 8);
            } else {
#pragma unroll
                for (int g = 0; g < 4; ++g) A.v[i][g] = f32x4{0.f, 0.f, 0.f, 0.f};
            }
        }
#pragma unroll
        for (int j = 0; j < TN; ++j) {
            if (wrow[j]) {
                const float* src = wrow[j] + (size_t)kt_next * BK;
#pragma unroll
                for (int g = 0; g < 4; ++g) Bf.v[j][g] = *reinterpret_cast<const f32x4*>(src + g * 8);
            } else {
#pragma unroll
                for (int g = 0; g < 4; ++g) Bf.v[j][g] = f32x4{0.f, 0.f, 0.f, 0.f};
            }
        }
        kt_next += KW;
        c0 += BK * KW;
        while (c0 >= p.Cin) {
            c0 -= p.Cin;
            if (++kw == p.KW) { kw = 0; ++kh; }
        }
    };

    f32x16 acc[TM][TN];
#pragma unroll
    for (int i = 0; i < TM; ++i)
#pragma unroll
        for (int j = 0; j < TN; ++j)
#pragma unroll
            for (int r = 0; r < 16; ++r) acc[i][j][r] = 0.f;

    auto compute = [&](const Frag<TM>& A, const Frag<TN>& Bf) {
#pragma unroll
        for (int g = 0; g < 4; ++g)
#pragma unroll
            for (int s = 0; s < 4; ++s)
#pragma unroll
                for (int i = 0; i < TM; ++i)
#pragma unroll
                    for (int j = 0; j < TN; ++j)
                        acc[i][j] = __builtin_amdgcn_mfma_f32_32x32x2f32(A.v[i][g][s], Bf.v[j][g][s], acc[i][j], 0, 0, 0);
    };

#pragma unroll
    for (int s = 0; s < D - 1; ++s)
        if (s < nt) load_tile(fa[s], fb[s]);
    for (int t = 0; t < nt; t += D) {
#pragma unroll
        for (int u = 0; u < D; ++u) {
            if (t + u < nt) {
                if (t + u + D - 1 < nt) load_tile(fa[(u + D - 1) % D], fb[(u + D - 1) % D]);
                compute(fa[u], fb[u]);
            }
        }
    }

    wave_tile_finish<TM, TN, KW, WPB>(p, smem, acc, wave, lane, tile_ok, tile_local, kslice, m0, n0);
}

template <int TM, int TN, int KW, int NS, int WPB = 4>
__global__ __launch_bounds__(WPB * 64) void conv_wdma_f32(const ConvP p) {
    static_assert(WPB % KW == 0 && WPB <= 4, "the K waves of a tile share a workgroup");
    constexpr int TPB = WPB / KW;
    constexpr int WM = 32 * TM, WN = 32 * TN;
    constexpr int AR = 4 * TM, BR = 4 * TN;
    constexpr int RP = 32;
    constexpr int STAGE = (WM + WN) * RP;
    constexpr int D = NS - 1;
    static_assert(NS >= 2 && NS <= 4 && (AR + BR) * D < 64, "ring depth / vmcnt field");
    static_assert((size_t)STAGE >= (size_t)WM * (WN + 4), "the finished tile is staged in the wave's first ring stage");
    extern __shared__ __attribute__((aligned(16))) float smem[];

    const int lane = threadIdx.x & 63;
    const int wave = __builtin_amdgcn_readfirstlane(threadIdx.x >> 6);
    const int tile_local = wave / KW, kslice = wave - tile_local * KW;
    const int frag_row = lane & 31, khalf = lane >> 5;
    YM_STAMP(0);
    constexpr bool TAIL = TM * TN == 1 && KW == 4 && WPB == 4;
    const bool in_tail = TAIL && (int)blockIdx.x >= p.main_blocks;
    int tile, tslice = 0, tsplit = 1;
    if (in_tail) {
        unsigned q, r;
        p.fd_tail.divmod(blockIdx.x - (unsigned)p.main_blocks, q, r);
        tile = p.main_tiles + (int)q; tslice = (int)r; tsplit = p.tail_split;
    } else {
        tile = ym_xcd_remap(blockIdx.x, TAIL ? p.main_blocks : (int)gridDim.x) * TPB + tile_local;
    }
    const bool tile_ok = tile < p.tiles_m * p.tiles_n;
    int tile_m = 0, tile_n = 0;
    if (tile_ok) ym_tile_decode(p, tile, tile_m, tile_n);
    const int m0 = tile_m * WM, n0 = tile_n * WN;
    const __amdgpu_buffer_rsrc_t rs_in = __builtin_amdgcn_make_buffer_rsrc((void*)p.in, 0, p.in_bytes, 0x00020000);
    const __amdgpu_buffer_rsrc_t rs_w = __builtin_amdgcn_make_buffer_rsrc((void*)p.w, 0, p.w_bytes, 0x00020000);

    const int drow = lane >> 3;
    int a_pix[AR], a_ih0[AR], a_iw0[AR];
    unsigned a_off[AR], wrow[BR];
#pragma unroll
    for (int i = 0; i < AR; ++i) {
        const int m = m0 + 8 * i + drow;
        if (tile_ok && m < p.M) {
            unsigned ub, urem, uoh, uow;
            p.fd_howo.divmod((unsigned)m, ub, urem);
            p.fd_wo.divmod(urem, uoh, uow);
            a_ih0[i] = (int)uoh * p.stride - p.pad;
            a_iw0[i] = (int)uow * p.stride - p.pad;
            a_pix[i] = ((int)ub * p.H + a_ih0[i]) * p.W + a_iw0[i];
        } else {
            a_ih0[i] = -(1 << 20); a_iw0[i] = -(1 << 20); a_pix[i] = 0;
        }
    }
#pragma unroll
    for (int j = 0; j < BR; ++j) {
        const int n = n0 + 8 * j + drow;
        const int c4 = (lane & 7) ^ ((4 * j + (lane >> 4)) & 7);
        wrow[j] = (tile_ok && n < p.Cout) ? (unsigned)((n * p.Kpad + c4 * 4) * 4) : p.w_bytes;
    }

    const int k_lo = in_tail ? tslice * p.tail_ktps : 0, k_hi = in_tail ? min(p.nkt, k_lo + p.tail_ktps) : p.nkt;
    const int per = (k_hi - k_lo + KW - 1) / KW;
    const int kt_beg = k_lo + kslice * per, kt_end = tile_ok ? min(k_hi, kt_beg + per) : kt_beg;
    const int nt = max(0, kt_end - kt_beg);
    int kh, kw, c0;
    {
        unsigned tap, uc0, ukh, ukw;
        p.fd_cin.divmod((unsigned)(kt_beg * BK), tap, uc0);
        p.fd_kw.divmod(tap, ukh, ukw);
        c0 = (int)uc0; kh = (int)ukh; kw = (int)ukw;
    }
    bool tap_dirty = true;
    int ld_kt = kt_beg;
    float* ring = smem + (size_t)wave * NS * STAGE;

    auto dma_next = [&](int stage) __attribute__((always_inline)) {
        typedef __attribute__((address_space(3))) void* lds_ptr;
        if (tap_dirty) {
            tap_dirty = false;
#pragma unroll
            for (int i = 0; i < AR; ++i) {
                const int ih = a_ih0[i] + kh, iw = a_iw0[i] + kw;
                const bool ok = (unsigned)ih < (unsigned)p.H && (unsigned)iw < (unsigned)p.W;
                const int c4 = (lane & 7) ^ ((4 * i + (lane >> 4)) & 7);
                a_off[i] = (unsigned)(((a_pix[i] + kh * p.W + kw) * p.Cin + c4 * 4) * 4) | (ok ? 0u : OOB);
            }
        }
        float* a = ring + stage * STAGE;
        float* b = a + WM * RP;
        const int soff_a = c0 * 4, soff_b = ld_kt * BK * 4;
#pragma unroll
        for (int i = 0; i < AR; ++i)
            __builtin_amdgcn_raw_ptr_buffer_load_lds(rs_in, (lds_ptr)(a + 8 * i * RP), 16, (int)a_off[i], soff_a, 0, 0);
#pragma unroll
        for (int j = 0; j < BR; ++j) {
            const unsigned wo = wrow[j];
            __builtin_amdgcn_raw_ptr_buffer_load_lds(rs_w, (lds_ptr)(b + 8 * j * RP), 16, (int)wo, soff_b, 0, 0);
        }
        ++ld_kt;
        c0 += BK;
        if (c0 >= p.Cin) {
            c0 = 0;
            if (++kw == p.KW) { kw = 0; ++kh; }
            tap_dirty = true;
        }
    };

    typedef const __attribute__((address_space(3))) f32x4* lds_frag_ptr;
    lds_frag_ptr pa[4], pb[4];
#pragma unroll
    for (int g = 0; g < 4; ++g) {
        const int goff = ((2 * g + khalf) ^ ((frag_row >> 1) & 7)) * 4;
        pa[g] = (lds_frag_ptr)(ring + frag_row * RP + goff);
        pb[g] = (lds_frag_ptr)(ring + WM * RP + frag_row * RP + goff);
    }
    f32x16 acc[TM][TN];
#pragma unroll
    for (int i = 0; i < TM; ++i)
#pragma unroll
        for (int j = 0; j < TN; ++j)
#pragma unroll
            for (int r = 0; r < 16; ++r) acc[i][j][r] = 0.f;
    constexpr bool DUAL = TM * TN == 1;
    f32x16 acc_odd;
#pragma unroll
    for (int r = 0; r < 16; ++r) acc_odd[r] = 0.f;

    auto compute = [&](auto S) __attribute__((always_inline)) {
        constexpr int ST = decltype(S)::value;
#pragma unroll
        for (int g = 0; g < 4; ++g) {
            f32x4 fa[TM], fb[TN];
#pragma unroll
            for (int i = 0; i < TM; ++i) fa[i] = pa[g][(ST * STAGE + i * 32 * RP) / 4];
#pragma unroll
            for (int j = 0; j < TN; ++j) fb[j] = pb[g][(ST * STAGE + j * 32 * RP) / 4];
#pragma unroll
            for (int s4 = 0; s4 < 4; ++s4) {
                if constexpr (DUAL) {
                    if (s4 & 1) acc_odd = __builtin_amdgcn_mfma_f32_32x32x2f32(fa[0][s4], fb[0][s4], acc_odd, 0, 0, 0);
                    else acc[0][0] = __builtin_amdgcn_mfma_f32_32x32x2f32(fa[0][s4], fb[0][s4], acc[0][0], 0, 0, 0);
                } else {
#pragma unroll
                    for (int i = 0; i < TM; ++i)
#pragma unroll
                        for (int j = 0; j < TN; ++j)
                            acc[i][j] = __builtin_amdgcn_mfma_f32_32x32x2f32(fa[i][s4], fb[j][s4], acc[i][j], 0, 0, 0);
                }
            }
        }
    };

    constexpr int WAIT = waitcnt_vm((AR + BR) * D) & ~(15 << 8);
#pragma unroll
    for (int d = 0; d < D; ++d) dma_next(d);
#ifdef YM_TRACE
    if (p.trace) { __builtin_amdgcn_s_waitcnt(waitcnt_vm((AR + BR) * (D - 1))); YM_STAMP(1); }
#endif
#ifdef YM_TRACE
    const int abl = p.bnb_relu;
#endif
    auto tile_step = [&](auto S) __attribute__((always_inline)) {
        constexpr int ST = decltype(S)::value;
        __builtin_amdgcn_sched_barrier(0);
#ifdef YM_TRACE
        if (abl >= 1 && abl <= 3) {
            if (abl == 1) {
                dma_next((ST + D) % NS);
                __builtin_amdgcn_s_waitcnt(WAIT);
            } else if (abl == 2) {
                compute(S);
            } else {
                const f32x4 ra = {1.f, 2.f, 3.f, 4.f}, rb = {.5f, .25f, .125f, 1.f};
#pragma unroll
                for (int g = 0; g < 4; ++g)
#pragma unroll
                    for (int s4 = 0; s4 < 4; ++s4) {
                        if constexpr (DUAL) {
                            if (s4 & 1) acc_odd = __builtin_amdgcn_mfma_f32_32x32x2f32(ra[s4], rb[s4], acc_odd, 0, 0, 0);
                            else acc[0][0] = __builtin_amdgcn_mfma_f32_32x32x2f32(ra[s4], rb[s4], acc[0][0], 0, 0, 0);
                        } else {
#pragma unroll
                            for (int i = 0; i < TM; ++i)
#pragma unroll
                                for (int j = 0; j < TN; ++j)
                                    acc[i][j] = __builtin_amdgcn_mfma_f32_32x32x2f32(ra[s4], rb[s4], acc[i][j], 0, 0, 0);
                        }
                    }
            }
        } else
#endif
        {
            dma_next((ST + D) % NS);
            __builtin_amdgcn_s_waitcnt(WAIT);
            compute(S);
        }
    };
    int t = 0;
    for (; t + NS <= nt; t += NS) static_for<0, NS>([&](auto S) __attribute__((always_inline)) { tile_step(S); });
    static_for<0, NS - 1>([&](auto S) __attribute__((always_inline)) { if (t + decltype(S)::value < nt) tile_step(S); });
    if constexpr (DUAL) acc[0][0] += acc_odd;
    YM_STAMP(2);
    asm volatile("s_waitcnt vmcnt(0) lgkmcnt(0)" ::: "memory");
    __syncthreads();
    if constexpr (TAIL) {
        if (in_tail) {
            constexpr int CP = WN + 4;
            float* mine = smem + (size_t)wave * WM * CP;
#pragma unroll
            for (int r = 0; r < 16; ++r) mine[(4 * khalf + (r & 3) + 8 * (r >> 2)) * CP + frag_row] = acc[0][0][r];
            __syncthreads();
            const int lt = threadIdx.x, col4 = lt & 7, row = lt >> 3;
            const int n = n0 + col4 * 4, m = m0 + row;
            f32x4 v = *reinterpret_cast<const f32x4*>(smem + row * CP + col4 * 4);
#pragma unroll
            for (int w2 = 1; w2 < KW; ++w2) v += *reinterpret_cast<const f32x4*>(smem + (size_t)w2 * WM * CP + row * CP + col4 * 4);
            const __amdgpu_buffer_rsrc_t rs_ws = __builtin_amdgcn_make_buffer_rsrc((void*)p.ws, 0, p.ws_bytes, 0x00020000);
            const unsigned sb = WM * WN * 4;
            const unsigned ws0 = (unsigned)(tile - p.main_tiles) * (unsigned)tsplit * sb + (unsigned)(row * WN + col4 * 4) * 4;
            buf_st16_sc1(rs_ws, ws0 + (unsigned)tslice * sb, v);
            asm volatile("s_waitcnt vmcnt(0)" ::: "memory");
            __syncthreads();
            int* s_last = reinterpret_cast<int*>(smem);
            if (lt == 0) {
                int* cnt = p.counters + tile;
                const int old = __hip_atomic_fetch_add(cnt, 1, __ATOMIC_RELAXED, __HIP_MEMORY_SCOPE_AGENT);
                *s_last = old == tsplit - 1;
                if (old == tsplit - 1) __hip_atomic_store(cnt, 0, __ATOMIC_RELAXED, __HIP_MEMORY_SCOPE_AGENT);
            }
            __syncthreads();
            if (*s_last && m < p.M && n < p.Cout) {
                f32x4 part[8];
#pragma unroll
                for (int s2 = 0; s2 < 8; ++s2) part[s2] = buf_ld16_sc1(rs_ws, s2 < tsplit ? ws0 + (unsigned)s2 * sb : OOB);
                f32x4 sum = part[0];
#pragma unroll
                for (int s2 = 1; s2 < 8; ++s2) if (s2 < tsplit) sum += part[s2];
                f32x4 sc = {1.f, 1.f, 1.f, 1.f}, sh = {0.f, 0.f, 0.f, 0.f};
                if (p.scale) sc = *reinterpret_cast<const f32x4*>(p.scale + n);
                if (p.shift) sh = *reinterpret_cast<const f32x4*>(p.shift + n);
                sum = __builtin_elementwise_fma(sum, sc, sh);
                if (p.residual) sum += *reinterpret_cast<const f32x4*>(p.residual + (size_t)m * p.Cout + n);
                const int act = p.seg[0].act;
#pragma unroll
                for (int e = 0; e < 4; ++e) sum[e] = ym_apply_act(sum[e], act);
                *reinterpret_cast<f32x4*>(p.seg[0].out + (size_t)m * p.Cout + n) = sum;
            }
            YM_STAMP(3);
            return;
        }
    }
    wave_tile_finish<TM, TN, KW, WPB>(p, smem, acc, wave, lane, tile_ok, tile_local, kslice, m0, n0);
    YM_STAMP(3);
}

template <int TM, int TN, int KW, int WPB>
int launch(ConvP p, hipStream_t st) {
    constexpr int TPB = WPB / KW;
    p.tiles_m = ym_cdiv(p.M, 32 * TM);
    p.tiles_n = ym_cdiv(p.Cout, 32 * TN);
    p.ksplit = 1;
    const int grid = ym_cdiv(p.tiles_m * p.tiles_n, TPB);
    const size_t lds = (size_t)WPB * 32 * TM * (32 * TN + 4) * sizeof(float);
    static YmLdsAttr attr = {};
    if (int rc = ym_ensure_dyn_lds(attr, reinterpret_cast<const void*>(conv_wave_f32<TM, TN, KW, WPB>), lds, "conv_wave_f32")) return rc;
    hipLaunchKernelGGL((conv_wave_f32<TM, TN, KW, WPB>), dim3(grid), dim3(WPB * 64), lds, st, p);
    return ym_check_launch("conv_wave_f32");
}

template <int TM, int TN>
int dispatch_kw(const ConvP& p, int kwaves, hipStream_t st) {
    switch (kwaves) {
        case 1: return launch<TM, TN, 1, 4>(p, st);
        case 2: return launch<TM, TN, 2, 4>(p, st);
        case 4: return launch<TM, TN, 4, 4>(p, st);
        case 8:
            if constexpr (TM * TN < 4) return launch<TM, TN, 8, 8>(p, st);
            [[fallthrough]];
        default: ym_set_error("conv(wave): unsupported kwaves %d for a %dx%d wave tile", kwaves, 32 * TM, 32 * TN); return YM_EINVAL;
    }
}

template <int TM, int TN, int KW, int NS, int WPB>
int launch_dma(ConvP p, hipStream_t st) {
    constexpr int TPB = WPB / KW;
    p.tiles_m = ym_cdiv(p.M, 32 * TM);
    p.tiles_n = ym_cdiv(p.Cout, 32 * TN);
    p.fd_tiles_n = FastDiv::make((unsigned)p.tiles_n);
    ym_set_tile_order(p, 0, true);
    p.ksplit = 1;
    int grid = ym_cdiv(p.tiles_m * p.tiles_n, TPB);
    if (TM * TN == 1 && KW == 4 && WPB == 4) {
        p.main_blocks = p.main_tiles;
        grid = p.main_tiles + (p.tiles_m * p.tiles_n - p.main_tiles) * p.tail_split;
    }
    const size_t lds = (size_t)WPB * NS * (32 * TM + 32 * TN) * 32 * sizeof(float);
    static YmLdsAttr attr = {};
    if (int rc = ym_ensure_dyn_lds(attr, reinterpret_cast<const void*>(conv_wdma_f32<TM, TN, KW, NS, WPB>), lds, "conv_wdma_f32")) return rc;
    hipLaunchKernelGGL((conv_wdma_f32<TM, TN, KW, NS, WPB>), dim3(grid), dim3(WPB * 64), lds, st, p);
    return ym_check_launch("conv_wdma_f32");
}

template <int TM, int TN>
int dispatch_dma(const ConvP& p, int kwaves, int ns, int wpb, hipStream_t st) {
    if (wpb <= 0) wpb = 4;
#define YM_DMA_CASE(KW_, NS_, WPB_) if (kwaves == KW_ && ns == NS_ && wpb == WPB_) return launch_dma<TM, TN, KW_, NS_, WPB_>(p, st)
    YM_DMA_CASE(1, 2, 4); YM_DMA_CASE(1, 3, 4); YM_DMA_CASE(2, 2, 4); YM_DMA_CASE(2, 3, 4); YM_DMA_CASE(4, 2, 4); YM_DMA_CASE(4, 3, 4);
    YM_DMA_CASE(1, 2, 1); YM_DMA_CASE(1, 3, 1); YM_DMA_CASE(1, 2, 2); YM_DMA_CASE(1, 3, 2); YM_DMA_CASE(2, 2, 2); YM_DMA_CASE(2, 3, 2);
    if constexpr (TM * TN == 1) { YM_DMA_CASE(1, 4, 4); YM_DMA_CASE(2, 4, 4); YM_DMA_CASE(4, 4, 4); YM_DMA_CASE(1, 4, 1); YM_DMA_CASE(1, 4, 2); }
#undef YM_DMA_CASE
    ym_set_error("conv(wave, DMA ring): kwaves %d, ring of %d, %d waves per workgroup is not built for a %dx%d wave tile", kwaves, ns, wpb, 32 * TM, 32 * TN);
    return YM_EINVAL;
}

}

int ym_launch_conv_wave(const ConvP& p, int tm, int tn, int kwaves, int ring, int wpb, hipStream_t st) {
    if (ring > 0) {
        if (tm == 32 && tn == 32) return dispatch_dma<1, 1>(p, kwaves, ring, wpb, st);
        if (tm == 64 && tn == 32) return dispatch_dma<2, 1>(p, kwaves, ring, wpb, st);
        if (tm == 32 && tn == 64) return dispatch_dma<1, 2>(p, kwaves, ring, wpb, st);
        ym_set_error("conv(wave, DMA ring): tile must be 32x32, 64x32 or 32x64, got %dx%d", tm, tn);
        return YM_EINVAL;
    }
    if (tm == 32 && tn == 32) return dispatch_kw<1, 1>(p, kwaves, st);
    if (tm == 64 && tn == 32) return dispatch_kw<2, 1>(p, kwaves, st);
    if (tm == 32 && tn == 64) return dispatch_kw<1, 2>(p, kwaves, st);
    if (tm == 64 && tn == 64) return dispatch_kw<2, 2>(p, kwaves, st);
    ym_set_error("conv(wave): tile must be 32/64 x 32/64, got %dx%d", tm, tn);
    return YM_EINVAL;
}
```

Measured before the change: 511.8 img/s.

## Compact wave-conv kernel arguments into a 256-byte hot struct with prefetch hints

Introduces a compact WaveArgs struct (exactly 256 bytes, four scalar loads) for the wave/DMA conv kernels, moving rarely used segment data to a separate kernarg fetched lazily, and reorders ConvP so hot fields come first. Inline asm forces early scalar loads of hot arguments, a fast path skips im2col index math for plain 1x1 convolutions, and scale/shift loads are hoisted before the tail reduction. The aim is to cut kernel-entry latency and per-thread index arithmetic in many small bs=1 convolutions. It adds ABI complexity and relies on the kernarg layout offset computation being correct.

```diff
diff --git a/yolact_minimal_amd/csrc/conv_common.h b/yolact_minimal_amd/csrc/conv_common.h
--- a/yolact_minimal_amd/csrc/conv_common.h
+++ b/yolact_minimal_amd/csrc/conv_common.h
@@ -48,10 +48,31 @@
 struct ConvP {
     const float* in;
     const float* w;
+    float* ws;
+    unsigned in_bytes, w_bytes, ws_bytes;
+    int main_blocks, main_tiles, tail_split, tail_ktps;
+    int ksplit, kt_per_split, nkt;
+    FastDiv fd_ksplit, fd_tail;
+    int n_groups;
+    FastDiv fd_grp, fd_gn, fd_gn_last;
+    int M, Cout, Kpad, Cin;
+    FastDiv fd_howo, fd_wo;
+    int stride, pad, H, W;
+    FastDiv fd_cin, fd_kw;
+    int KH, KW;
+    int total_items;
+    int vec;
     const float* scale;
     const float* shift;
     const float* residual;
-    float* ws;
+    int* counters;
+    int M_pix;
+    int nseg;
+    SegDev seg[3];
+    int B, Ho, Wo, HoWo, tiles_m, tiles_n;
+    FastDiv fd_tiles_n;
+    int bn_ordered;
+    int bnb_relu;
     double* bn_sum;
     double* bn_sumsq;
     const float* bnb_y;
@@ -60,39 +81,63 @@
     const float* bnb_invstd;
     const float* bnb_gamma;
     const float* bnb_beta;
-    int bnb_relu;
-    int bn_ordered;
-    int* counters;
-    int B, H, W, Cin, Cout, KH, KW, stride, pad, Ho, Wo, Kpad;
-    int M, HoWo, nkt, ksplit, kt_per_split, tiles_m, tiles_n;
-    int main_blocks, main_tiles, tail_split, tail_ktps;
-    FastDiv fd_ksplit, fd_tail, fd_tiles_n, fd_howo, fd_wo, fd_cin, fd_kw;
     int nlev;
     int lev_h[5], lev_w[5], lev_m[6], lev_pix[6];
     int cls;
-    int M_pix;
     int cls_tile0[5];
     int cls_rows[4];
     int cls_w[4];
     FastDiv cls_fd_hw[4], cls_fd_w[4];
     int cls_kh0[4], cls_kw0[4], cls_nkw[4];
     int cls_nkt[4], cls_ktps[4], cls_tail_ktps[4];
-    int n_groups;
-    FastDiv fd_grp, fd_gn, fd_gn_last;
     long long* trace;
     const int* trace_epoch;
     int trace_ring;
     int trace_stride;
     int trace_rt;
     int* trace_hw;
-    unsigned in_bytes, w_bytes, ws_bytes;
-    int total_items;
+    long long* trace_entry;
+};
+
+struct WaveHot {
+    const float* in;
+    const float* w;
+    unsigned in_bytes, w_bytes;
+    int main_tiles, ntiles;
+    FastDiv fd_tail;
+    int n_groups;
+    FastDiv fd_grp, fd_gn, fd_gn_last;
+    int M, Cout;
+    int fast1x1;
+    unsigned cin_bytes, kpad_bytes;
+    FastDiv fd_howo, fd_wo;
+    int stride, pad, H, W;
+    int nkt, tail_ktps;
+    FastDiv fd_cin, fd_kw;
+    const float* residual;
+    const float* scale;
+    const float* shift;
+    float* out;
+    float* ws;
+    int* counters;
+    unsigned res_bytes, ws_bytes;
+    int vec, act;
+    int remap_n;
+    unsigned reserved_[3];
+};
+static_assert(sizeof(WaveHot) == 256, "WaveHot: four 64-byte scalar loads");
+struct WaveArgs : WaveHot {
+#ifdef YM_TRACE
+    long long* trace; const int* trace_epoch; int trace_ring, trace_stride, trace_rt, abl; int* trace_hw; long long* trace_entry;
+#endif
+};
+struct WaveSegs {
     int nseg;
-    int vec;
     SegDev seg[3];
 };
 
-__device__ __forceinline__ void ym_tile_decode(const ConvP& p, int id, int& tile_m, int& tile_n) {
+template <class P>
+__device__ __forceinline__ void ym_tile_decode(const P& p, int id, int& tile_m, int& tile_n) {
     const unsigned g = p.fd_grp.div((unsigned)id);
     const unsigned r = (unsigned)id - g * p.fd_grp.d;
     const bool last = (int)g == p.n_groups - 1;
@@ -129,15 +174,44 @@
     p.fd_grp = FastDiv::make((unsigned)(tm * gw));
 }
 
+#define YM_FD_(f) "s"(p.f.mg), "s"(p.f.sh), "s"(p.f.d)
+__device__ __forceinline__ void ym_fetch_wave_args(const WaveArgs& p) {
+    asm volatile("" :: "s"(p.in), "s"(p.w), "s"(p.in_bytes), "s"(p.w_bytes), "s"(p.main_tiles), "s"(p.ntiles), YM_FD_(fd_tail), "s"(p.n_groups),
+                 YM_FD_(fd_grp), YM_FD_(fd_gn), YM_FD_(fd_gn_last), "s"(p.M), "s"(p.Cout), "s"(p.fast1x1), "s"(p.cin_bytes), "s"(p.kpad_bytes),
+                 YM_FD_(fd_howo), YM_FD_(fd_wo));
+    asm volatile("" :: "s"(p.stride), "s"(p.pad), "s"(p.H), "s"(p.W), "s"(p.nkt), "s"(p.tail_ktps), "s"(p.remap_n), YM_FD_(fd_cin), YM_FD_(fd_kw),
+                 "s"(p.residual), "s"(p.scale), "s"(p.shift), "s"(p.out), "s"(p.ws), "s"(p.counters), "s"(p.res_bytes), "s"(p.ws_bytes),
+                 "s"(p.vec), "s"(p.act));
+}
+__device__ __forceinline__ void ym_fetch_conv_hot(const ConvP& p) {
+    asm volatile("" :: "s"(p.in), "s"(p.w), "s"(p.ws), "s"(p.in_bytes), "s"(p.w_bytes), "s"(p.ws_bytes), "s"(p.main_blocks), "s"(p.main_tiles),
+                 "s"(p.tail_split), "s"(p.tail_ktps), "s"(p.ksplit), "s"(p.kt_per_split), "s"(p.nkt), YM_FD_(fd_ksplit), YM_FD_(fd_tail),
+                 "s"(p.n_groups), YM_FD_(fd_grp), YM_FD_(fd_gn), YM_FD_(fd_gn_last));
+    asm volatile("" :: "s"(p.M), "s"(p.Cout), "s"(p.Kpad), "s"(p.Cin), YM_FD_(fd_howo), YM_FD_(fd_wo), "s"(p.stride), "s"(p.pad), "s"(p.H), "s"(p.W),
+                 YM_FD_(fd_cin), YM_FD_(fd_kw), "s"(p.KH), "s"(p.KW), "s"(p.vec), "s"(p.scale), "s"(p.shift), "s"(p.residual));
+}
+#undef YM_FD_
+__device__ __forceinline__ const WaveSegs* ym_wave_segs() {
+    constexpr size_t off = (sizeof(WaveArgs) + alignof(WaveSegs) - 1) / alignof(WaveSegs) * alignof(WaveSegs);
+    const char* q = (const char*)__builtin_amdgcn_kernarg_segment_ptr() + off;
+    asm volatile("" : "+s"(q));
+    return reinterpret_cast<const WaveSegs*>(q);
+}
+
 #ifdef YM_TRACE
-__device__ __forceinline__ size_t ym_trace_region(const ConvP& p) {
+template <class P>
+__device__ __forceinline__ size_t ym_trace_region(const P& p) {
     if (!p.trace_epoch) return 0;
     const unsigned e = (unsigned)__hip_atomic_load(p.trace_epoch, __ATOMIC_RELAXED, __HIP_MEMORY_SCOPE_AGENT);
     return (size_t)(e % (unsigned)p.trace_ring) * (p.trace_stride ? (unsigned)p.trace_stride : gridDim.x);
 }
 #define YM_STAMP(i) do { if ((i) == 3) __builtin_amdgcn_s_waitcnt(0); if (p.trace && threadIdx.x == 0) { const size_t reg_ = ym_trace_region(p); p.trace[(reg_ + blockIdx.x) * 4 + (i)] = (long long)((p.trace_epoch || p.trace_rt) ? __builtin_amdgcn_s_memrealtime() : __builtin_amdgcn_s_memtime()) | ((i) == 0 ? (long long)(__builtin_amdgcn_s_getreg(0x1814) & 15) << 60 : 0ll); if ((i) == 0 && p.trace_hw) p.trace_hw[reg_ + blockIdx.x] = (int)__builtin_amdgcn_s_getreg(0xF804); } } while (0)
+#define YM_ENTRY_STAMP() const long long entry_rt_ = (long long)__builtin_amdgcn_s_memrealtime(), entry_t_ = (long long)__builtin_amdgcn_s_memtime(); __builtin_amdgcn_sched_barrier(0)
+#define YM_STAMP_ENTRY_STORE() do { if (p.trace && p.trace_entry && threadIdx.x == 0) p.trace_entry[ym_trace_region(p) + blockIdx.x] = (p.trace_epoch || p.trace_rt) ? entry_rt_ : entry_t_; } while (0)
 #else
 #define YM_STAMP(i) do { } while (0)
+#define YM_ENTRY_STAMP() do { } while (0)
+#define YM_STAMP_ENTRY_STORE() do { } while (0)
 #endif
 
 
diff --git a/yolact_minimal_amd/csrc/conv_mfma.hip b/yolact_minimal_amd/csrc/conv_mfma.hip
--- a/yolact_minimal_amd/csrc/conv_mfma.hip
+++ b/yolact_minimal_amd/csrc/conv_mfma.hip
@@ -11,6 +11,7 @@
 template <int BM, int BN, int MODE, int NS, bool DL = false, bool PF = false, bool RG = false, int SPL = 0>
 __global__ __launch_bounds__(256) void conv_igemm_f32(const ConvP p) {
     static_assert(SPL == 0 || (SPL <= 3 && !DL && !PF && (NS == 2 || NS == 3) && MODE != 1), "split-bf16: register staging, Cin % 32 == 0");
+    ym_fetch_conv_hot(p);
     constexpr int LB = SPL ? 2 : NS;
     constexpr int TM = BM / 64, TN = BN / 64;
     constexpr int AR = BM / 32, BR = BN / 32;
@@ -876,7 +877,7 @@
     p.bn_sum = d->bn_sum; p.bn_sumsq = d->bn_sumsq; p.bn_ordered = (d->bn_sum && d->bn_ordered) ? 1 : 0;
     p.bnb_y = d->bnb_y; p.bnb_out = d->bnb_out; p.bnb_mean = d->bnb_mean; p.bnb_invstd = d->bnb_invstd;
     p.bnb_gamma = d->bnb_gamma; p.bnb_beta = d->bnb_beta; p.bnb_relu = d->bnb_relu;
-    p.trace = nullptr; p.trace_epoch = nullptr; p.trace_ring = 0; p.trace_stride = 0; p.trace_rt = 0; p.trace_hw = nullptr;
+    p.trace = nullptr; p.trace_epoch = nullptr; p.trace_ring = 0; p.trace_stride = 0; p.trace_rt = 0; p.trace_hw = nullptr; p.trace_entry = nullptr;
 #ifdef YM_TRACE
     if (const char* e = getenv("YM_TRACE_PTR")) p.trace = (long long*)strtoull(e, nullptr, 10);
     if (const char* e = getenv("YM_TRACE_EPOCH_PTR")) p.trace_epoch = (const int*)strtoull(e, nullptr, 10);
@@ -884,6 +885,7 @@
     if (const char* e = getenv("YM_TRACE_GRID")) p.trace_stride = atoi(e);
     if (const char* e = getenv("YM_TRACE_REALTIME")) p.trace_rt = atoi(e);
     if (const char* e = getenv("YM_TRACE_HW_PTR")) p.trace_hw = (int*)strtoull(e, nullptr, 10);
+    if (const char* e = getenv("YM_TRACE_ENTRY_PTR")) p.trace_entry = (long long*)strtoull(e, nullptr, 10);
     if (p.trace_ring <= 0) p.trace_epoch = nullptr;
     if (const char* e = getenv("YM_PERS_ABL")) { if (!d->bn_sum) p.bnb_relu = atoi(e); }
 #endif
diff --git a/yolact_minimal_amd/csrc/conv_persist.hip b/yolact_minimal_amd/csrc/conv_persist.hip
--- a/yolact_minimal_amd/csrc/conv_persist.hip
+++ b/yolact_minimal_amd/csrc/conv_persist.hip
@@ -15,6 +15,7 @@
     static_assert(BM == 64 && BN == 64, "the accumulator staging aliases one ring stage: (BM + BN) * 128 B == BM * BN * 4 B");
     static_assert(MODE == 0 || MODE == 2, "Cin % 32 == 0 convolution / data gradient");
     static_assert(NS >= 2 && NS <= 12, "ring depth");
+    ym_fetch_conv_hot(p);
     constexpr int AR = BM / 32, BR = BN / 32;
     constexpr int RP = 32;
     constexpr int D = NS - 1;
diff --git a/yolact_minimal_amd/csrc/conv_wave.hip b/yolact_minimal_amd/csrc/conv_wave.hip
--- a/yolact_minimal_amd/csrc/conv_wave.hip
+++ b/yolact_minimal_amd/csrc/conv_wave.hip
@@ -11,18 +11,40 @@
     f32x4 v[N][4];
 };
 
+__device__ __forceinline__ void wave_epilogue_store(const WaveArgs& p, const WaveSegs& sg, int m, int n, float acc) {
+    float v = acc;
+    v = __builtin_fmaf(v, p.scale ? p.scale[n] : 1.f, p.shift ? p.shift[n] : 0.f);
+    if (p.residual) v += p.residual[(size_t)m * p.Cout + n];
+    const int b = (int)p.fd_howo.div((unsigned)m), pix = m - b * (int)p.fd_howo.d;
+#pragma unroll
+    for (int s = 0; s < 3; ++s) {
+        if (s < sg.nseg && n >= sg.seg[s].n0 && n < sg.seg[s].n1) {
+            const SegDev& g = sg.seg[s];
+            g.out[(size_t)b * g.bstride + (size_t)pix * g.pitch + (n - g.n0)] = ym_apply_act(v, g.act);
+        }
+    }
+}
+
 template <int TM, int TN, int KW, int WPB>
-__device__ __forceinline__ void wave_tile_finish(const ConvP& p, float* slabs, f32x16 (&acc)[TM][TN], int wave, int lane, bool tile_ok,
-                                                 int tile_local, int kslice, int m0, int n0) {
+__device__ __forceinline__ void wave_tile_finish(const WaveArgs& p, float* slabs, f32x16 (&acc)[TM][TN], int wave, int lane,
+                                                 bool tile_ok, int tile_local, int kslice, int m0, int n0) {
     constexpr int WM = 32 * TM, WN = 32 * TN;
     constexpr int CP = WN + 4;
     const int frag_row = lane & 31, khalf = lane >> 5;
     constexpr int C4_ = WN / 4, LANES_ = KW * 64, NPASS = (WM * C4_ + LANES_ - 1) / LANES_;
     f32x4 pre_res[NPASS];
+    f32x4 sc = {1.f, 1.f, 1.f, 1.f}, sh = {0.f, 0.f, 0.f, 0.f};
+    if (p.vec && tile_ok) {
+        const int n_ = n0 + ((kslice * 64 + lane) % C4_) * 4;
+        if (n_ < p.Cout) {
+            if (p.scale) sc = *reinterpret_cast<const f32x4*>(p.scale + n_);
+            if (p.shift) sh = *reinterpret_cast<const f32x4*>(p.shift + n_);
+        }
+    }
     const bool pre = p.vec && p.residual != nullptr && tile_ok;
     if (pre) {
         const int lt_ = kslice * 64 + lane, col4_ = lt_ % C4_, row0_ = lt_ / C4_;
-        const __amdgpu_buffer_rsrc_t rs_res = __builtin_amdgcn_make_buffer_rsrc((void*)p.residual, 0, (unsigned)((size_t)p.M * p.Cout * 4), 0x00020000);
+        const __amdgpu_buffer_rsrc_t rs_res = __builtin_amdgcn_make_buffer_rsrc((void*)p.residual, 0, p.res_bytes, 0x00020000);
 #pragma unroll
         for (int k = 0; k < NPASS; ++k) {
             const int m = m0 + row0_ + k * (LANES_ / C4_), n = n0 + col4_ * 4;
@@ -47,10 +69,7 @@
         const int col4 = lt % C4, row0 = lt / C4;
         const int n = n0 + col4 * 4;
         if (n < p.Cout) {
-            f32x4 sc = {1.f, 1.f, 1.f, 1.f}, sh = {0.f, 0.f, 0.f, 0.f};
-            if (p.scale) sc = *reinterpret_cast<const f32x4*>(p.scale + n);
-            if (p.shift) sh = *reinterpret_cast<const f32x4*>(p.shift + n);
-            const int act = p.seg[0].act;
+            const int act = p.act;
 #pragma unroll
             for (int k = 0; k < NPASS; ++k) {
                 const int row = row0 + k * (LANES / C4);
@@ -63,10 +82,11 @@
                 if (p.residual) v += pre_res[k];
 #pragma unroll
                 for (int e = 0; e < 4; ++e) v[e] = ym_apply_act(v[e], act);
-                *reinterpret_cast<f32x4*>(p.seg[0].out + (size_t)m * p.Cout + n) = v;
+                *reinterpret_cast<f32x4*>(p.out + (size_t)m * p.Cout + n) = v;
             }
         }
     } else {
+        const WaveSegs& sg = *ym_wave_segs();
         for (int e = lt; e < WM * WN; e += LANES) {
             const int row = e / WN, col = e - row * WN;
             const int m = m0 + row, n = n0 + col;
@@ -74,14 +94,15 @@
                 float v = slab0[row * CP + col];
 #pragma unroll
                 for (int s = 1; s < KW; ++s) v += slab0[(size_t)s * WM * CP + row * CP + col];
-                epilogue_store(p, m, n, v);
+                wave_epilogue_store(p, sg, m, n, v);
             }
         }
     }
 }
 
 template <int TM, int TN, int KW, int WPB>
-__global__ __launch_bounds__(WPB * 64) void conv_wave_f32(const ConvP p) {
+__global__ __launch_bounds__(WPB * 64) void conv_wave_f32(const WaveArgs p, const WaveSegs) {
+    ym_fetch_wave_args(p);
     constexpr int TPB = WPB / KW;
     constexpr int WM = 32 * TM, WN = 32 * TN;
     constexpr int D = 3;
@@ -92,23 +113,29 @@
     const int tile_local = wave / KW, kslice = wave - tile_local * KW;
     const int frag_row = lane & 31, khalf = lane >> 5;
 
-    const int bid = ym_xcd_remap(blockIdx.x, gridDim.x);
+    const int bid = ym_xcd_remap(blockIdx.x, p.remap_n);
     const int tile = bid * TPB + tile_local;
-    const int ntiles = p.tiles_m * p.tiles_n;
-    const bool tile_ok = tile < ntiles;
-    const int tile_m = tile_ok ? tile / p.tiles_n : 0, tile_n = tile_ok ? tile - tile_m * p.tiles_n : 0;
+    const bool tile_ok = tile < p.ntiles;
+    int tile_m = 0, tile_n = 0;
+    if (tile_ok) ym_tile_decode(p, tile, tile_m, tile_n);
     const int m0 = tile_m * WM, n0 = tile_n * WN;
+    const int Cin = (int)p.fd_cin.d, KW_ = (int)p.fd_kw.d;
 
     int a_pix[TM], a_ih0[TM], a_iw0[TM];
 #pragma unroll
     for (int i = 0; i < TM; ++i) {
         const int m = m0 + i * 32 + frag_row;
         if (tile_ok && m < p.M) {
-            const int b = m / p.HoWo, rem = m - b * p.HoWo;
-            const int oh = rem / p.Wo, ow = rem - oh * p.Wo;
-            a_ih0[i] = oh * p.stride - p.pad;
-            a_iw0[i] = ow * p.stride - p.pad;
-            a_pix[i] = (b * p.H + a_ih0[i]) * p.W + a_iw0[i];
+            if (p.fast1x1) {
+                a_ih0[i] = 0; a_iw0[i] = 0; a_pix[i] = m;
+            } else {
+                unsigned ub, urem, uoh, uow;
+                p.fd_howo.divmod((unsigned)m, ub, urem);
+                p.fd_wo.divmod(urem, uoh, uow);
+                a_ih0[i] = (int)uoh * p.stride - p.pad;
+                a_iw0[i] = (int)uow * p.stride - p.pad;
+                a_pix[i] = ((int)ub * p.H + a_ih0[i]) * p.W + a_iw0[i];
+            }
         } else {
             a_ih0[i] = -(1 << 20); a_iw0[i] = -(1 << 20); a_pix[i] = 0;
         }
@@ -117,17 +144,16 @@
 #pragma unroll
     for (int j = 0; j < TN; ++j) {
         const int n = n0 + j * 32 + frag_row;
-        wrow[j] = (tile_ok && n < p.Cout) ? p.w + (size_t)n * p.Kpad + khalf * 4 : nullptr;
+        wrow[j] = (tile_ok && n < p.Cout) ? p.w + (size_t)n * (p.kpad_bytes / 4) + khalf * 4 : nullptr;
     }
 
     const int nt = tile_ok ? (p.nkt - kslice + KW - 1) / KW : 0;
     int kh, kw, c0;
     {
-        const int k0 = kslice * BK;
-        const int tap = k0 / p.Cin;
-        c0 = k0 - tap * p.Cin;
-        kh = tap / p.KW;
-        kw = tap - kh * p.KW;
+        unsigned tap, uc0, ukh, ukw;
+        p.fd_cin.divmod((unsigned)(kslice * BK), tap, uc0);
+        p.fd_kw.divmod(tap, ukh, ukw);
+        c0 = (int)uc0; kh = (int)ukh; kw = (int)ukw;
     }
     int kt_next = kslice;
 
@@ -140,7 +166,7 @@
             const int ih = a_ih0[i] + kh, iw = a_iw0[i] + kw;
             const bool ok = (unsigned)ih < (unsigned)p.H && (unsigned)iw < (unsigned)p.W;
             if (ok) {
-                const float* src = p.in + (size_t)(a_pix[i] + tap_off) * p.Cin + c0 + khalf * 4;
+                const float* src = p.in + (size_t)(a_pix[i] + tap_off) * Cin + c0 + khalf * 4;
 #pragma unroll
                 for (int g = 0; g < 4; ++g) A.v[i][g] = *reinterpret_cast<const f32x4*>(src + g * 8);
             } else {
@@ -161,9 +187,9 @@
         }
         kt_next += KW;
         c0 += BK * KW;
-        while (c0 >= p.Cin) {
-            c0 -= p.Cin;
-            if (++kw == p.KW) { kw = 0; ++kh; }
+        while (c0 >= Cin) {
+            c0 -= Cin;
+            if (++kw == KW_) { kw = 0; ++kh; }
         }
     };
 
@@ -204,7 +230,9 @@
 }
 
 template <int TM, int TN, int KW, int NS, int WPB = 4>
-__global__ __launch_bounds__(WPB * 64) void conv_wdma_f32(const ConvP p) {
+__global__ __launch_bounds__(WPB * 64) void conv_wdma_f32(const WaveArgs p, const WaveSegs) {
+    YM_ENTRY_STAMP();
+    ym_fetch_wave_args(p);
     static_assert(WPB % KW == 0 && WPB <= 4, "the K waves of a tile share a workgroup");
     constexpr int TPB = WPB / KW;
     constexpr int WM = 32 * TM, WN = 32 * TN;
@@ -221,17 +249,18 @@
     const int tile_local = wave / KW, kslice = wave - tile_local * KW;
     const int frag_row = lane & 31, khalf = lane >> 5;
     YM_STAMP(0);
+    YM_STAMP_ENTRY_STORE();
     constexpr bool TAIL = TM * TN == 1 && KW == 4 && WPB == 4;
-    const bool in_tail = TAIL && (int)blockIdx.x >= p.main_blocks;
+    const bool in_tail = TAIL && (int)blockIdx.x >= p.main_tiles;
     int tile, tslice = 0, tsplit = 1;
     if (in_tail) {
         unsigned q, r;
-        p.fd_tail.divmod(blockIdx.x - (unsigned)p.main_blocks, q, r);
-        tile = p.main_tiles + (int)q; tslice = (int)r; tsplit = p.tail_split;
+        p.fd_tail.divmod(blockIdx.x - (unsigned)p.main_tiles, q, r);
+        tile = p.main_tiles + (int)q; tslice = (int)r; tsplit = (int)p.fd_tail.d;
     } else {
-        tile = ym_xcd_remap(blockIdx.x, TAIL ? p.main_blocks : (int)gridDim.x) * TPB + tile_local;
-    }
-    const bool tile_ok = tile < p.tiles_m * p.tiles_n;
+        tile = ym_xcd_remap(blockIdx.x, p.remap_n) * TPB + tile_local;
+    }
+    const bool tile_ok = tile < p.ntiles;
     int tile_m = 0, tile_n = 0;
     if (tile_ok) ym_tile_decode(p, tile, tile_m, tile_n);
     const int m0 = tile_m * WM, n0 = tile_n * WN;
@@ -239,41 +268,53 @@
     const __amdgpu_buffer_rsrc_t rs_w = __builtin_amdgcn_make_buffer_rsrc((void*)p.w, 0, p.w_bytes, 0x00020000);
 
     const int drow = lane >> 3;
+    const bool fast = p.fast1x1 != 0;
+    const int Cin = (int)p.fd_cin.d, KW_ = (int)p.fd_kw.d;
     int a_pix[AR], a_ih0[AR], a_iw0[AR];
     unsigned a_off[AR], wrow[BR];
-#pragma unroll
-    for (int i = 0; i < AR; ++i) {
-        const int m = m0 + 8 * i + drow;
-        if (tile_ok && m < p.M) {
-            unsigned ub, urem, uoh, uow;
-            p.fd_howo.divmod((unsigned)m, ub, urem);
-            p.fd_wo.divmod(urem, uoh, uow);
-            a_ih0[i] = (int)uoh * p.stride - p.pad;
-            a_iw0[i] = (int)uow * p.stride - p.pad;
-            a_pix[i] = ((int)ub * p.H + a_ih0[i]) * p.W + a_iw0[i];
-        } else {
-            a_ih0[i] = -(1 << 20); a_iw0[i] = -(1 << 20); a_pix[i] = 0;
-        }
-    }
 #pragma unroll
     for (int j = 0; j < BR; ++j) {
         const int n = n0 + 8 * j + drow;
         const int c4 = (lane & 7) ^ ((4 * j + (lane >> 4)) & 7);
-        wrow[j] = (tile_ok && n < p.Cout) ? (unsigned)((n * p.Kpad + c4 * 4) * 4) : p.w_bytes;
+        wrow[j] = (tile_ok && n < p.Cout) ? (unsigned)n * p.kpad_bytes + (unsigned)(c4 * 16) : p.w_bytes;
+    }
+    if (fast) {
+#pragma unroll
+        for (int i = 0; i < AR; ++i) {
+            const int m = m0 + 8 * i + drow;
+            const int c4 = (lane & 7) ^ ((4 * i + (lane >> 4)) & 7);
+            a_off[i] = (tile_ok && m < p.M) ? (unsigned)m * p.cin_bytes + (unsigned)(c4 * 16) : OOB;
+            a_pix[i] = 0; a_ih0[i] = 0; a_iw0[i] = 0;
+        }
+    } else {
+#pragma unroll
+        for (int i = 0; i < AR; ++i) {
+            const int m = m0 + 8 * i + drow;
+            if (tile_ok && m < p.M) {
+                unsigned ub, urem, uoh, uow;
+                p.fd_howo.divmod((unsigned)m, ub, urem);
+                p.fd_wo.divmod(urem, uoh, uow);
+                a_ih0[i] = (int)uoh * p.stride - p.pad;
+                a_iw0[i] = (int)uow * p.stride - p.pad;
+                a_pix[i] = ((int)ub * p.H + a_ih0[i]) * p.W + a_iw0[i];
+            } else {
+                a_ih0[i] = -(1 << 20); a_iw0[i] = -(1 << 20); a_pix[i] = 0;
+            }
+        }
     }
 
     const int k_lo = in_tail ? tslice * p.tail_ktps : 0, k_hi = in_tail ? min(p.nkt, k_lo + p.tail_ktps) : p.nkt;
     const int per = (k_hi - k_lo + KW - 1) / KW;
     const int kt_beg = k_lo + kslice * per, kt_end = tile_ok ? min(k_hi, kt_beg + per) : kt_beg;
     const int nt = max(0, kt_end - kt_beg);
-    int kh, kw, c0;
-    {
+    int kh = 0, kw = 0, c0 = kt_beg * BK;
+    if (!fast) {
         unsigned tap, uc0, ukh, ukw;
         p.fd_cin.divmod((unsigned)(kt_beg * BK), tap, uc0);
         p.fd_kw.divmod(tap, ukh, ukw);
         c0 = (int)uc0; kh = (int)ukh; kw = (int)ukw;
     }
-    bool tap_dirty = true;
+    bool tap_dirty = !fast;
     int ld_kt = kt_beg;
     float* ring = smem + (size_t)wave * NS * STAGE;
 
@@ -286,7 +327,7 @@
                 const int ih = a_ih0[i] + kh, iw = a_iw0[i] + kw;
                 const bool ok = (unsigned)ih < (unsigned)p.H && (unsigned)iw < (unsigned)p.W;
                 const int c4 = (lane & 7) ^ ((4 * i + (lane >> 4)) & 7);
-                a_off[i] = (unsigned)(((a_pix[i] + kh * p.W + kw) * p.Cin + c4 * 4) * 4) | (ok ? 0u : OOB);
+                a_off[i] = ((unsigned)(a_pix[i] + kh * p.W + kw) * p.cin_bytes + (unsigned)(c4 * 16)) | (ok ? 0u : OOB);
             }
         }
         float* a = ring + stage * STAGE;
@@ -302,9 +343,9 @@
         }
         ++ld_kt;
         c0 += BK;
-        if (c0 >= p.Cin) {
+        if (!fast && c0 >= Cin) {
             c0 = 0;
-            if (++kw == p.KW) { kw = 0; ++kh; }
+            if (++kw == KW_) { kw = 0; ++kh; }
             tap_dirty = true;
         }
     };
@@ -361,7 +402,7 @@
     if (p.trace) { __builtin_amdgcn_s_waitcnt(waitcnt_vm((AR + BR) * (D - 1))); YM_STAMP(1); }
 #endif
 #ifdef YM_TRACE
-    const int abl = p.bnb_relu;
+    const int abl = p.abl;
 #endif
     auto tile_step = [&](auto S) __attribute__((always_inline)) {
         constexpr int ST = decltype(S)::value;
@@ -409,12 +450,17 @@
     if constexpr (TAIL) {
         if (in_tail) {
             constexpr int CP = WN + 4;
+            const int lt = threadIdx.x, col4 = lt & 7, row = lt >> 3;
+            const int n = n0 + col4 * 4, m = m0 + row;
+            f32x4 sc = {1.f, 1.f, 1.f, 1.f}, sh = {0.f, 0.f, 0.f, 0.f};
+            if (m < p.M && n < p.Cout) {
+                if (p.scale) sc = *reinterpret_cast<const f32x4*>(p.scale + n);
+                if (p.shift) sh = *reinterpret_cast<const f32x4*>(p.shift + n);
+            }
             float* mine = smem + (size_t)wave * WM * CP;
 #pragma unroll
             for (int r = 0; r < 16; ++r) mine[(4 * khalf + (r & 3) + 8 * (r >> 2)) * CP + frag_row] = acc[0][0][r];
             __syncthreads();
-            const int lt = threadIdx.x, col4 = lt & 7, row = lt >> 3;
-            const int n = n0 + col4 * 4, m = m0 + row;
             f32x4 v = *reinterpret_cast<const f32x4*>(smem + row * CP + col4 * 4);
 #pragma unroll
             for (int w2 = 1; w2 < KW; ++w2) v += *reinterpret_cast<const f32x4*>(smem + (size_t)w2 * WM * CP + row * CP + col4 * 4);
@@ -439,15 +485,12 @@
                 f32x4 sum = part[0];
 #pragma unroll
                 for (int s2 = 1; s2 < 8; ++s2) if (s2 < tsplit) sum += part[s2];
-                f32x4 sc = {1.f, 1.f, 1.f, 1.f}, sh = {0.f, 0.f, 0.f, 0.f};
-                if (p.scale) sc = *reinterpret_cast<const f32x4*>(p.scale + n);
-                if (p.shift) sh = *reinterpret_cast<const f32x4*>(p.shift + n);
                 sum = __builtin_elementwise_fma(sum, sc, sh);
                 if (p.residual) sum += *reinterpret_cast<const f32x4*>(p.residual + (size_t)m * p.Cout + n);
-                const int act = p.seg[0].act;
+                const int act = p.act;
 #pragma unroll
                 for (int e = 0; e < 4; ++e) sum[e] = ym_apply_act(sum[e], act);
-                *reinterpret_cast<f32x4*>(p.seg[0].out + (size_t)m * p.Cout + n) = sum;
+                *reinterpret_cast<f32x4*>(p.out + (size_t)m * p.Cout + n) = sum;
             }
             YM_STAMP(3);
             return;
@@ -455,6 +498,31 @@
     }
     wave_tile_finish<TM, TN, KW, WPB>(p, smem, acc, wave, lane, tile_ok, tile_local, kslice, m0, n0);
     YM_STAMP(3);
+}
+
+void make_wave_args(const ConvP& p, int remap_n, WaveArgs& a, WaveSegs& sg) {
+    a.in = p.in; a.w = p.w; a.in_bytes = p.in_bytes; a.w_bytes = p.w_bytes;
+    a.main_tiles = p.main_tiles; a.ntiles = p.tiles_m * p.tiles_n;
+    a.fd_tail = p.fd_tail;
+    a.n_groups = p.n_groups; a.fd_grp = p.fd_grp; a.fd_gn = p.fd_gn; a.fd_gn_last = p.fd_gn_last;
+    a.M = p.M; a.Cout = p.Cout;
+    a.fast1x1 = p.KH == 1 && p.KW == 1 && p.stride == 1 && p.pad == 0 && p.Kpad == p.Cin && p.Ho == p.H && p.Wo == p.W;
+    a.cin_bytes = (unsigned)p.Cin * 4u; a.kpad_bytes = (unsigned)p.Kpad * 4u;
+    a.fd_howo = p.fd_howo; a.fd_wo = p.fd_wo;
+    a.stride = p.stride; a.pad = p.pad; a.H = p.H; a.W = p.W;
+    a.nkt = p.nkt; a.tail_ktps = p.tail_ktps;
+    a.fd_cin = p.fd_cin; a.fd_kw = p.fd_kw;
+    a.residual = p.residual; a.scale = p.scale; a.shift = p.shift; a.out = p.seg[0].out;
+    a.ws = p.ws; a.counters = p.counters;
+    a.res_bytes = (unsigned)((size_t)p.M * p.Cout * 4); a.ws_bytes = p.ws_bytes;
+    a.vec = p.vec; a.act = p.seg[0].act; a.remap_n = remap_n;
+    for (unsigned& r : a.reserved_) r = 0;
+#ifdef YM_TRACE
+    a.trace = p.trace; a.trace_epoch = p.trace_epoch; a.trace_ring = p.trace_ring; a.trace_stride = p.trace_stride;
+    a.trace_rt = p.trace_rt; a.abl = p.bnb_relu; a.trace_hw = p.trace_hw; a.trace_entry = p.trace_entry;
+#endif
+    sg.nseg = p.nseg;
+    for (int i = 0; i < 3; ++i) sg.seg[i] = p.seg[i];
 }
 
 template <int TM, int TN, int KW, int WPB>
@@ -462,12 +530,15 @@
     constexpr int TPB = WPB / KW;
     p.tiles_m = ym_cdiv(p.M, 32 * TM);
     p.tiles_n = ym_cdiv(p.Cout, 32 * TN);
-    p.ksplit = 1;
+    ym_set_tile_order(p, 1, false);
     const int grid = ym_cdiv(p.tiles_m * p.tiles_n, TPB);
     const size_t lds = (size_t)WPB * 32 * TM * (32 * TN + 4) * sizeof(float);
     static YmLdsAttr attr = {};
     if (int rc = ym_ensure_dyn_lds(attr, reinterpret_cast<const void*>(conv_wave_f32<TM, TN, KW, WPB>), lds, "conv_wave_f32")) return rc;
-    hipLaunchKernelGGL((conv_wave_f32<TM, TN, KW, WPB>), dim3(grid), dim3(WPB * 64), lds, st, p);
+    WaveArgs a;
+    WaveSegs sg;
+    make_wave_args(p, grid, a, sg);
+    hipLaunchKernelGGL((conv_wave_f32<TM, TN, KW, WPB>), dim3(grid), dim3(WPB * 64), lds, st, a, sg);
     return ym_check_launch("conv_wave_f32");
 }
 
@@ -489,18 +560,17 @@
     constexpr int TPB = WPB / KW;
     p.tiles_m = ym_cdiv(p.M, 32 * TM);
     p.tiles_n = ym_cdiv(p.Cout, 32 * TN);
-    p.fd_tiles_n = FastDiv::make((unsigned)p.tiles_n);
     ym_set_tile_order(p, 0, true);
-    p.ksplit = 1;
     int grid = ym_cdiv(p.tiles_m * p.tiles_n, TPB);
-    if (TM * TN == 1 && KW == 4 && WPB == 4) {
-        p.main_blocks = p.main_tiles;
+    if (TM * TN == 1 && KW == 4 && WPB == 4)
         grid = p.main_tiles + (p.tiles_m * p.tiles_n - p.main_tiles) * p.tail_split;
-    }
     const size_t lds = (size_t)WPB * NS * (32 * TM + 32 * TN) * 32 * sizeof(float);
     static YmLdsAttr attr = {};
     if (int rc = ym_ensure_dyn_lds(attr, reinterpret_cast<const void*>(conv_wdma_f32<TM, TN, KW, NS, WPB>), lds, "conv_wdma_f32")) return rc;
-    hipLaunchKernelGGL((conv_wdma_f32<TM, TN, KW, NS, WPB>), dim3(grid), dim3(WPB * 64), lds, st, p);
+    WaveArgs a;
+    WaveSegs sg;
+    make_wave_args(p, TM * TN == 1 && KW == 4 && WPB == 4 ? p.main_tiles : grid, a, sg);
+    hipLaunchKernelGGL((conv_wdma_f32<TM, TN, KW, NS, WPB>), dim3(grid), dim3(WPB * 64), lds, st, a, sg);
     return ym_check_launch("conv_wdma_f32");
 }
 
```

New measurement: 524.2 img/s, median of 6. +2.4%, better.
